# fgladwin/rocJPEG

Measured on NVIDIA B200. Metric: decoded_MP_per_s_rocJpegDecodeBatched, higher is better.
Workload: dtype u8 / int16 coefficients / int32 IDCT / fp32 colour

## Files before the change

### include/rocjpeg_b200_ext.h

```cpp
#ifndef ROCJPEG_B200_EXT_H
#define ROCJPEG_B200_EXT_H

#include <stddef.h>
#include <stdint.h>

#include "rocjpeg.h"

#if defined(__cplusplus)
extern "C" {
#endif

#define ROCJPEG_B200_STAGE_COUNT 7

typedef struct {
    float stage_ms[ROCJPEG_B200_STAGE_COUNT];
    float total_ms;
    uint32_t sync_rounds;
    uint32_t decodes_per_round[8];
    uint64_t scan_bytes;
    uint64_t blocks;
    uint64_t subsequences;
    uint64_t plane_bytes;
    uint64_t output_bytes;
    uint64_t h2d_bytes, d2h_bytes;
    uint32_t kernel_launches;
    int32_t subsequence_bytes;
    int32_t lanes;
    float host_submit_ms;
    float host_wait_ms;
    int32_t devices;
    uint64_t entries;
    uint32_t truncated_images;
    uint32_t pad_;
    uint64_t fused_blocks;
} RocJpegB200Stats;

RocJpegStatus rocJpegB200SetProfiling(RocJpegHandle handle, int enable);
RocJpegStatus rocJpegB200GetStats(RocJpegHandle handle, RocJpegB200Stats *stats);

RocJpegStatus rocJpegB200Prepare(RocJpegHandle handle, RocJpegStreamHandle *jpeg_stream_handles, int batch_size,
                                 const RocJpegDecodeParams *decode_params, RocJpegImage *destinations);
RocJpegStatus rocJpegB200Run(RocJpegHandle handle);

RocJpegStatus rocJpegB200GetScaledImageInfo(RocJpegHandle handle, RocJpegStreamHandle jpeg_stream_handle, int scale_denom, uint8_t *num_components,
                                            RocJpegChromaSubsampling *subsampling, uint32_t *widths, uint32_t *heights);
RocJpegStatus rocJpegB200DecodeBatchedScaled(RocJpegHandle handle, RocJpegStreamHandle *jpeg_stream_handles, int batch_size,
                                             const RocJpegDecodeParams *decode_params, const int32_t *scale_denoms, RocJpegImage *destinations);
RocJpegStatus rocJpegB200PrepareScaled(RocJpegHandle handle, RocJpegStreamHandle *jpeg_stream_handles, int batch_size,
                                       const RocJpegDecodeParams *decode_params, const int32_t *scale_denoms, RocJpegImage *destinations);

RocJpegStatus rocJpegB200ParseAndDecodeBatched(RocJpegHandle handle, RocJpegStreamHandle *jpeg_stream_handles,
                                               const unsigned char *const *datas, const size_t *lengths, int batch_size,
                                               const RocJpegDecodeParams *decode_params, RocJpegImage *destinations,
                                               double *parse_seconds);

RocJpegStatus rocJpegB200StreamLoadFiles(RocJpegStreamHandle *jpeg_stream_handles, const char *const *paths, int count,
                                         int io_threads, RocJpegStatus *per_file_status);

RocJpegStatus rocJpegB200GetCoefficients(RocJpegHandle handle, int index, int16_t *host_out, size_t count);
RocJpegStatus rocJpegB200GetPlanes(RocJpegHandle handle, int index, uint8_t *host_out, size_t count);

typedef struct {
    uint32_t segments_seen;
    uint32_t scan_size;
    uint32_t flags;
    uint32_t reserved;
} RocJpegB200ScanStatus;
#define ROCJPEG_B200_SCAN_NO_EOI 1u
#define ROCJPEG_B200_SCAN_STRAY_MARKER 2u
#define ROCJPEG_B200_SCAN_EXTRA_RESTARTS 4u
#define ROCJPEG_B200_SCAN_MISSING_INTERVALS 8u
#define ROCJPEG_B200_SCAN_EMPTY_INTERVAL 16u
#define ROCJPEG_B200_DECODE_SHORT 32u
#define ROCJPEG_B200_TRUNCATED_MASK (8u | 16u | 32u)
RocJpegStatus rocJpegB200GetScanStatus(RocJpegHandle handle, int index, RocJpegB200ScanStatus *status);
RocJpegStatus rocJpegB200GetImageStatus(RocJpegHandle handle, int index, uint32_t *flags);
RocJpegStatus rocJpegB200GetDeviceSegment(RocJpegHandle handle, int index, uint32_t segment, uint8_t *host_out, size_t capacity,
                                          uint32_t *nbytes);

typedef struct {
    int32_t width, height, num_components, chroma_subsampling;
    int32_t h_sampling[3], v_sampling[3], quant_selector[3], dc_selector[3], ac_selector[3];
    int32_t restart_interval;
    uint32_t num_mcus;
    uint32_t scan_offset;
    uint32_t raw_bytes;
    int32_t mcus_x, mcus_y, blocks_per_mcu;
    int32_t blocks_w[3], blocks_h[3];
    uint32_t num_segments;
    int32_t decode_status;
    int32_t source_is_device_visible;
    int32_t source_is_zero_copy;
    int32_t features;
} RocJpegB200StreamInfo;
#define ROCJPEG_B200_FEAT_SOF1 1
#define ROCJPEG_B200_FEAT_DQT16 2
#define ROCJPEG_B200_FEAT_HUFF_ID23 4
RocJpegStatus rocJpegB200StreamGetInfo(RocJpegStreamHandle jpeg_stream_handle, RocJpegB200StreamInfo *info);
typedef struct {
    uint32_t scan_size;
    uint32_t restart_markers_seen;
    uint32_t num_segments;
    uint64_t clean_bytes;
} RocJpegB200HostScanInfo;
RocJpegStatus rocJpegB200StreamHostScan(RocJpegStreamHandle jpeg_stream_handle, RocJpegB200HostScanInfo *info);
RocJpegStatus rocJpegB200StreamGetSegment(RocJpegStreamHandle jpeg_stream_handle, uint32_t segment, uint8_t *out,
                                          size_t capacity, uint32_t *nbytes);
RocJpegStatus rocJpegB200StreamGetLastError(RocJpegStreamHandle jpeg_stream_handle, char *out, size_t capacity);
RocJpegStatus rocJpegB200StreamGetQuantTable(RocJpegStreamHandle jpeg_stream_handle, int id, uint16_t out_natural[64]);
RocJpegStatus rocJpegB200StreamGetHuffmanTable(RocJpegStreamHandle jpeg_stream_handle, int is_ac, int id, uint8_t bits[16],
                                               uint8_t vals[256], uint32_t *count);

RocJpegStatus rocJpegB200PlanShards(const uint64_t *cost, int batch_size, int num_devices, int *out_device);
RocJpegStatus rocJpegB200PlanShardsPinned(const uint64_t *cost, const int *fixed, int batch_size, int num_devices, int *out_device);
RocJpegStatus rocJpegB200GetDeviceCount(RocJpegHandle handle, int *num_devices);

const char *rocJpegB200Version(void);
// ... 6 lines not shown
```

### rocjpeg_b200/api.py

```python
from __future__ import annotations

import ctypes as C
import os

HERE = os.path.dirname(os.path.abspath(__file__))
LIB_PATH = os.environ.get("ROCJPEG_B200_LIB") or os.path.join(HERE, "lib", "librocjpeg.so")

STATUS = {
    0: "ROCJPEG_STATUS_SUCCESS", -1: "ROCJPEG_STATUS_NOT_INITIALIZED", -2: "ROCJPEG_STATUS_INVALID_PARAMETER",
    -3: "ROCJPEG_STATUS_BAD_JPEG", -4: "ROCJPEG_STATUS_JPEG_NOT_SUPPORTED", -5: "ROCJPEG_STATUS_OUTOF_MEMORY",
    -6: "ROCJPEG_STATUS_EXECUTION_FAILED", -7: "ROCJPEG_STATUS_ARCH_MISMATCH", -8: "ROCJPEG_STATUS_INTERNAL_ERROR",
    -9: "ROCJPEG_STATUS_IMPLEMENTATION_NOT_SUPPORTED", -10: "ROCJPEG_STATUS_HW_JPEG_DECODER_NOT_SUPPORTED",
    -11: "ROCJPEG_STATUS_RUNTIME_ERROR", -12: "ROCJPEG_STATUS_NOT_IMPLEMENTED",
}
SUCCESS, NOT_INITIALIZED, INVALID_PARAMETER, BAD_JPEG, JPEG_NOT_SUPPORTED = 0, -1, -2, -3, -4
EXECUTION_FAILED, RUNTIME_ERROR, NOT_IMPLEMENTED = -6, -11, -12
CSS_444, CSS_440, CSS_422, CSS_420, CSS_411, CSS_400, CSS_UNKNOWN = 0, 1, 2, 3, 4, 5, -1
CSS_NAME = {0: "444", 1: "440", 2: "422", 3: "420", 4: "411", 5: "400", -1: "unknown"}
OUTPUT_NATIVE, OUTPUT_YUV_PLANAR, OUTPUT_Y, OUTPUT_RGB, OUTPUT_RGB_PLANAR = 0, 1, 2, 3, 4
FMT = {"native": 0, "yuv_planar": 1, "y": 2, "rgb": 3, "rgb_planar": 4}
BACKEND_HARDWARE, BACKEND_HYBRID = 0, 1
STAGES = ("upload", "destuff", "huffman_sync", "huffman_write", "dc", "idct", "output")


class RocJpegImage(C.Structure):
    _fields_ = [("channel", C.c_void_p * 4), ("pitch", C.c_uint32 * 4)]


class _Crop(C.Structure):
    _fields_ = [("left", C.c_int16), ("top", C.c_int16), ("right", C.c_int16), ("bottom", C.c_int16)]


class _Target(C.Structure):
    _fields_ = [("width", C.c_uint32), ("height", C.c_uint32)]


class RocJpegDecodeParams(C.Structure):
    _fields_ = [("output_format", C.c_int), ("crop_rectangle", _Crop), ("target_dimension", _Target)]


class Stats(C.Structure):
    _fields_ = [
        ("stage_ms", C.c_float * 7), ("total_ms", C.c_float), ("sync_rounds", C.c_uint32),
        ("decodes_per_round", C.c_uint32 * 8), ("scan_bytes", C.c_uint64), ("blocks", C.c_uint64),
        ("subsequences", C.c_uint64), ("plane_bytes", C.c_uint64), ("output_bytes", C.c_uint64),
        ("h2d_bytes", C.c_uint64), ("d2h_bytes", C.c_uint64), ("kernel_launches", C.c_uint32),
        ("subsequence_bytes", C.c_int32), ("lanes", C.c_int32),
        ("host_submit_ms", C.c_float), ("host_wait_ms", C.c_float), ("devices", C.c_int32),
        ("entries", C.c_uint64), ("truncated_images", C.c_uint32), ("pad_", C.c_uint32), ("fused_blocks", C.c_uint64),
    ]


class StreamInfo(C.Structure):
    _fields_ = [
        ("width", C.c_int32), ("height", C.c_int32), ("num_components", C.c_int32), ("chroma_subsampling", C.c_int32),
        ("h_sampling", C.c_int32 * 3), ("v_sampling", C.c_int32 * 3), ("quant_selector", C.c_int32 * 3),
        ("dc_selector", C.c_int32 * 3), ("ac_selector", C.c_int32 * 3), ("restart_interval", C.c_int32),
        ("num_mcus", C.c_uint32), ("scan_offset", C.c_uint32), ("raw_bytes", C.c_uint32),
        ("mcus_x", C.c_int32), ("mcus_y", C.c_int32), ("blocks_per_mcu", C.c_int32),
        ("blocks_w", C.c_int32 * 3), ("blocks_h", C.c_int32 * 3), ("num_segments", C.c_uint32),
        ("decode_status", C.c_int32), ("source_is_device_visible", C.c_int32), ("source_is_zero_copy", C.c_int32),
        ("features", C.c_int32),
    ]


class ScanStatus(C.Structure):
    _fields_ = [("segments_seen", C.c_uint32), ("scan_size", C.c_uint32), ("flags", C.c_uint32), ("reserved", C.c_uint32)]


FEAT_SOF1, FEAT_DQT16, FEAT_HUFF_ID23 = 1, 2, 4
SCAN_NO_EOI, SCAN_STRAY_MARKER, SCAN_EXTRA_RESTARTS, SCAN_MISSING_INTERVALS, SCAN_EMPTY_INTERVAL = 1, 2, 4, 8, 16
DECODE_SHORT, TRUNCATED_MASK = 32, 8 | 16 | 32


class HostScanInfo(C.Structure):
    _fields_ = [("scan_size", C.c_uint32), ("restart_markers_seen", C.c_uint32), ("num_segments", C.c_uint32),
                ("clean_bytes", C.c_uint64)]


EXPORTS = (
    "rocJpegStreamCreate", "rocJpegStreamParse", "rocJpegStreamDestroy", "rocJpegCreate", "rocJpegDestroy",
    "rocJpegGetImageInfo", "rocJpegDecode", "rocJpegDecodeBatched", "rocJpegGetErrorName",
)
EXT_EXPORTS = (
    "rocJpegB200SetProfiling", "rocJpegB200GetStats", "rocJpegB200Prepare", "rocJpegB200Run",
    "rocJpegB200GetCoefficients", "rocJpegB200GetPlanes", "rocJpegB200StreamGetInfo", "rocJpegB200StreamGetSegment",
    "rocJpegB200StreamGetQuantTable", "rocJpegB200StreamGetHuffmanTable", "rocJpegB200Version", "rocJpegB200StreamGetLastError",
    "rocJpegB200PlanShards", "rocJpegB200GetDeviceCount", "rocJpegB200StreamHostScan",
    "rocJpegB200GetScanStatus", "rocJpegB200GetDeviceSegment", "rocJpegB200ParseAndDecodeBatched",
    "rocJpegB200PlanShardsPinned", "rocJpegB200GetImageStatus", "rocJpegB200StreamLoadFiles",
    "rocJpegB200GetScaledImageInfo", "rocJpegB200DecodeBatchedScaled", "rocJpegB200PrepareScaled",
)
SCALES = (1, 2, 4, 8)

_lib = None


class RocJpegError(RuntimeError):
    def __init__(self, status: int, where: str):
        self.status = status
        super().__init__(f"{where}: {STATUS.get(status, status)}")


def load_library() -> C.CDLL:
    global _lib
    if _lib is not None:
        return _lib
    if not os.path.exists(LIB_PATH):
        raise RuntimeError(
            f"{LIB_PATH} is missing: build it with `make -C rocjpeg_b200/csrc` (or __graft_entry__.build()). "
            "rocjpeg_b200 has no CPU fallback.")
    L = C.CDLL(LIB_PATH)
    vp, i32 = C.c_void_p, C.c_int
    L.rocJpegStreamCreate.argtypes = [C.POINTER(vp)]
    L.rocJpegStreamParse.argtypes = [vp, C.c_size_t, vp]
    L.rocJpegStreamDestroy.argtypes = [vp]
    L.rocJpegCreate.argtypes = [i32, i32, C.POINTER(vp)]
    L.rocJpegDestroy.argtypes = [vp]
    L.rocJpegGetImageInfo.argtypes = [vp, vp, C.POINTER(C.c_uint8), C.POINTER(i32), C.POINTER(C.c_uint32), C.POINTER(C.c_uint32)]
    L.rocJpegDecode.argtypes = [vp, vp, C.POINTER(RocJpegDecodeParams), C.POINTER(RocJpegImage)]
    L.rocJpegDecodeBatched.argtypes = [vp, C.POINTER(vp), i32, C.POINTER(RocJpegDecodeParams), C.POINTER(RocJpegImage)]
    L.rocJpegGetErrorName.argtypes = [i32]
    L.rocJpegGetErrorName.restype = C.c_char_p
    L.rocJpegB200SetProfiling.argtypes = [vp, i32]
    L.rocJpegB200GetStats.argtypes = [vp, C.POINTER(Stats)]
    L.rocJpegB200Prepare.argtypes = [vp, C.POINTER(vp), i32, C.POINTER(RocJpegDecodeParams), C.POINTER(RocJpegImage)]
    L.rocJpegB200Run.argtypes = [vp]
    L.rocJpegB200GetScaledImageInfo.argtypes = [vp, vp, i32, C.POINTER(C.c_uint8), C.POINTER(i32), C.POINTER(C.c_uint32), C.POINTER(C.c_uint32)]
    L.rocJpegB200DecodeBatchedScaled.argtypes = [vp, C.POINTER(vp), i32, C.POINTER(RocJpegDecodeParams), C.POINTER(C.c_int32), C.POINTER(RocJpegImage)]
    L.rocJpegB200PrepareScaled.argtypes = [vp, C.POINTER(vp), i32, C.POINTER(RocJpegDecodeParams), C.POINTER(C.c_int32), C.POINTER(RocJpegImage)]
    L.rocJpegB200GetCoefficients.argtypes = [vp, i32, vp, C.c_size_t]
    L.rocJpegB200GetPlanes.argtypes = [vp, i32, vp, C.c_size_t]
# ... 287 lines not shown
```

### rocjpeg_b200/csrc/api.cpp

```cpp
#include <algorithm>
#include <atomic>
#include <chrono>
#include <thread>
#include <cstring>
#include <exception>
#include <iostream>
#include <memory>
#include <string>
#include <vector>

#include "decoder.h"
#include "jpeg_parser.h"
#include "rocjpeg_b200_ext.h"

#define ERR(X) std::cerr << "[ERR] " << " {" << __func__ << "} " << " " << X << std::endl;

namespace {

struct StreamHandle {
    std::shared_ptr<rjb::StreamParser> parser = std::make_shared<rjb::StreamParser>();
    std::string error;
};

struct DecoderHandle {
// ... 159 lines not shown
        ERR(e.what());
        return ROCJPEG_STATUS_RUNTIME_ERROR;
    }
}

RocJpegStatus ROCJPEGAPI rocJpegDecodeBatched(RocJpegHandle handle, RocJpegStreamHandle* jpeg_stream_handles, int batch_size,
                                              const RocJpegDecodeParams* decode_params, RocJpegImage* destinations) {
    return rocJpegB200DecodeBatchedScaled(handle, jpeg_stream_handles, batch_size, decode_params, nullptr, destinations);
}

RocJpegStatus rocJpegB200DecodeBatchedScaled(RocJpegHandle handle, RocJpegStreamHandle* jpeg_stream_handles, int batch_size,
                                             const RocJpegDecodeParams* decode_params, const int32_t* scale_denoms, RocJpegImage* destinations) {
    if (handle == nullptr || jpeg_stream_handles == nullptr || decode_params == nullptr || destinations == nullptr)
        return ROCJPEG_STATUS_INVALID_PARAMETER;
    auto h = static_cast<DecoderHandle*>(handle);
    try {
        if (batch_size < 0) return ROCJPEG_STATUS_INVALID_PARAMETER;
        std::vector<const rjb::StreamParser*> streams;
        int st = CollectStreams(jpeg_stream_handles, batch_size, &streams);
        if (st != 0) return RocJpegStatus(st);
        std::vector<rjb::DestImage> dsts;
        st = ToDests(destinations, batch_size, scale_denoms, &dsts);
        if (st != 0) return RocJpegStatus(st);
        st = h->decoder->Decode(streams.data(), batch_size, ToParams(decode_params), dsts.data());
        if (st != 0) h->CaptureError(h->decoder->last_error());
        return RocJpegStatus(st);
    } catch (const std::exception& e) {
        h->CaptureError(e.what());
        ERR(e.what());
        return ROCJPEG_STATUS_RUNTIME_ERROR;
    }
}

const char* ROCJPEGAPI rocJpegGetErrorName(RocJpegStatus rocjpeg_status) {
    switch (rocjpeg_status) {
        case ROCJPEG_STATUS_SUCCESS: return "ROCJPEG_STATUS_SUCCESS";
        case ROCJPEG_STATUS_NOT_INITIALIZED: return "ROCJPEG_STATUS_NOT_INITIALIZED";
        case ROCJPEG_STATUS_INVALID_PARAMETER: return "ROCJPEG_STATUS_INVALID_PARAMETER";
        case ROCJPEG_STATUS_BAD_JPEG: return "ROCJPEG_STATUS_BAD_JPEG";
        case ROCJPEG_STATUS_JPEG_NOT_SUPPORTED: return "ROCJPEG_STATUS_JPEG_NOT_SUPPORTED";
        case ROCJPEG_STATUS_EXECUTION_FAILED: return "ROCJPEG_STATUS_EXECUTION_FAILED";
        case ROCJPEG_STATUS_ARCH_MISMATCH: return "ROCJPEG_STATUS_ARCH_MISMATCH";
        case ROCJPEG_STATUS_INTERNAL_ERROR: return "ROCJPEG_STATUS_INTERNAL_ERROR";
        case ROCJPEG_STATUS_IMPLEMENTATION_NOT_SUPPORTED: return "ROCJPEG_STATUS_IMPLEMENTATION_NOT_SUPPORTED";
        case ROCJPEG_STATUS_HW_JPEG_DECODER_NOT_SUPPORTED: return "ROCJPEG_STATUS_HW_JPEG_DECODER_NOT_SUPPORTED";
        case ROCJPEG_STATUS_RUNTIME_ERROR: return "ROCJPEG_STATUS_RUNTIME_ERROR";
        case ROCJPEG_STATUS_OUTOF_MEMORY: return "ROCJPEG_STATUS_OUTOF_MEMORY";
        case ROCJPEG_STATUS_NOT_IMPLEMENTED: return "ROCJPEG_STATUS_NOT_IMPLEMENTED";
        default: return "UNKNOWN_ERROR";
    }
}


RocJpegStatus rocJpegB200SetProfiling(RocJpegHandle handle, int enable) {
    if (handle == nullptr) return ROCJPEG_STATUS_INVALID_PARAMETER;
    static_cast<DecoderHandle*>(handle)->decoder->SetProfiling(enable);
    return ROCJPEG_STATUS_SUCCESS;
}

RocJpegStatus rocJpegB200GetStats(RocJpegHandle handle, RocJpegB200Stats* stats) {
    if (handle == nullptr || stats == nullptr) return ROCJPEG_STATUS_INVALID_PARAMETER;
    const rjb::BatchStats& s = static_cast<DecoderHandle*>(handle)->decoder->stats();
    std::memset(stats, 0, sizeof(*stats));
    for (int i = 0; i < ROCJPEG_B200_STAGE_COUNT; i++) stats->stage_ms[i] = s.stage_ms[i];
    stats->total_ms = s.total_ms;
    stats->sync_rounds = s.sync_rounds;
    for (int i = 0; i < 8; i++) stats->decodes_per_round[i] = s.decodes_per_round[i];
    stats->scan_bytes = s.scan_bytes;
    stats->blocks = s.blocks;
    stats->subsequences = s.subsequences;
    stats->plane_bytes = s.plane_bytes;
    stats->output_bytes = s.output_bytes;
    stats->h2d_bytes = s.h2d_bytes;
    stats->d2h_bytes = s.d2h_bytes;
    stats->kernel_launches = s.kernel_launches;
    stats->subsequence_bytes = s.sub_bytes;
    stats->lanes = s.lanes;
    stats->host_submit_ms = s.host_submit_ms;
    stats->host_wait_ms = s.host_wait_ms;
    stats->devices = s.devices;
    stats->entries = s.entries;
    stats->truncated_images = s.truncated_images;
    stats->fused_blocks = s.fused_blocks;
    return ROCJPEG_STATUS_SUCCESS;
}

RocJpegStatus rocJpegB200Prepare(RocJpegHandle handle, RocJpegStreamHandle* jpeg_stream_handles, int batch_size,
                                 const RocJpegDecodeParams* decode_params, RocJpegImage* destinations) {
    return rocJpegB200PrepareScaled(handle, jpeg_stream_handles, batch_size, decode_params, nullptr, destinations);
}

RocJpegStatus rocJpegB200PrepareScaled(RocJpegHandle handle, RocJpegStreamHandle* jpeg_stream_handles, int batch_size,
                                       const RocJpegDecodeParams* decode_params, const int32_t* scale_denoms, RocJpegImage* destinations) {
    if (handle == nullptr || jpeg_stream_handles == nullptr || decode_params == nullptr || destinations == nullptr || batch_size <= 0)
        return ROCJPEG_STATUS_INVALID_PARAMETER;
    auto h = static_cast<DecoderHandle*>(handle);
    try {
        std::vector<const rjb::StreamParser*> streams;
        int st = CollectStreams(jpeg_stream_handles, batch_size, &streams);
        if (st != 0) return RocJpegStatus(st);
        std::vector<rjb::DestImage> dsts;
        st = ToDests(destinations, batch_size, scale_denoms, &dsts);
        if (st != 0) return RocJpegStatus(st);
        return RocJpegStatus(h->decoder->Prepare(streams.data(), batch_size, ToParams(decode_params), dsts.data()));
    } catch (const std::exception& e) {
        h->CaptureError(e.what());
        ERR(e.what());
        return ROCJPEG_STATUS_RUNTIME_ERROR;
    }
}

RocJpegStatus rocJpegB200Run(RocJpegHandle handle) {
    if (handle == nullptr) return ROCJPEG_STATUS_INVALID_PARAMETER;
    auto h = static_cast<DecoderHandle*>(handle);
    try {
        return RocJpegStatus(h->decoder->Run());
    } catch (const std::exception& e) {
        h->CaptureError(e.what());
        ERR(e.what());
        return ROCJPEG_STATUS_RUNTIME_ERROR;
    }
}

RocJpegStatus rocJpegB200ParseAndDecodeBatched(RocJpegHandle handle, RocJpegStreamHandle* jpeg_stream_handles, const unsigned char* const* datas,
                                               const size_t* lengths, int batch_size, const RocJpegDecodeParams* decode_params,
                                               RocJpegImage* destinations, double* parse_seconds) {
    if (handle == nullptr || jpeg_stream_handles == nullptr || datas == nullptr || lengths == nullptr || batch_size < 0)
        return ROCJPEG_STATUS_INVALID_PARAMETER;
    const auto t0 = std::chrono::steady_clock::now();
    for (int i = 0; i < batch_size; i++) {
        const RocJpegStatus st = rocJpegStreamParse(datas[i], lengths[i], jpeg_stream_handles[i]);
        if (st != ROCJPEG_STATUS_SUCCESS) return st;
    }
    if (parse_seconds) *parse_seconds = std::chrono::duration<double>(std::chrono::steady_clock::now() - t0).count();
    return rocJpegDecodeBatched(handle, jpeg_stream_handles, batch_size, decode_params, destinations);
}

RocJpegStatus rocJpegB200StreamLoadFiles(RocJpegStreamHandle* jpeg_stream_handles, const char* const* paths, int count, int io_threads,
                                         RocJpegStatus* per_file_status) {
    if (jpeg_stream_handles == nullptr || paths == nullptr || count < 0) return ROCJPEG_STATUS_INVALID_PARAMETER;
    for (int i = 0; i < count; i++)
        if (jpeg_stream_handles[i] == nullptr || paths[i] == nullptr) return ROCJPEG_STATUS_INVALID_PARAMETER;
    const int nthreads = std::max(1, std::min(io_threads <= 0 ? 8 : io_threads, std::max(count, 1)));
    std::vector<RocJpegStatus> status(size_t(count), ROCJPEG_STATUS_SUCCESS);
    std::atomic<int> next{0};
    auto work = [&]() {
        for (;;) {
            const int i = next.fetch_add(1, std::memory_order_relaxed);
            if (i >= count) return;
            auto h = static_cast<StreamHandle*>(jpeg_stream_handles[i]);
            try {
                const int rc = h->parser->ParseFile(paths[i]);
                h->error = rc == 0 ? std::string() : h->parser->last_error();
                status[size_t(i)] = rc == 0 ? ROCJPEG_STATUS_SUCCESS : rc == -2 ? ROCJPEG_STATUS_INVALID_PARAMETER : ROCJPEG_STATUS_BAD_JPEG;
            } catch (const std::exception& e) {
                h->error = e.what();
                status[size_t(i)] = ROCJPEG_STATUS_RUNTIME_ERROR;
            }
        }
    };
    std::vector<std::thread> pool;
    for (int t = 1; t < nthreads; t++) pool.emplace_back(work);
    work();
    for (auto& t : pool) t.join();
    RocJpegStatus first = ROCJPEG_STATUS_SUCCESS;
    for (int i = 0; i < count; i++) {
// ... 150 lines not shown
```

### rocjpeg_b200/csrc/decoder.cpp

```cpp
#include "decoder.h"

#include "huff_core.cuh"

#include <cuda_runtime.h>

#include <algorithm>
#include <chrono>
#include <cstdint>
#include <cstdio>
#include <cstdlib>
#include <cstring>
#include <iostream>

namespace rjb {

namespace {
constexpr int kSuccess = 0, kNotInitialized = -1, kInvalidParameter = -2, kBadJpeg = -3, kNotSupported = -4,
              kOutOfMemory = -5, kExecutionFailed = -6, kNotImplemented = -12;

inline size_t AlignUp(size_t v, size_t a) { return (v + a - 1) / a * a; }

int EnvInt(const char* name, int dflt) {
    const char* v = std::getenv(name);
    return (v && *v) ? std::atoi(v) : dflt;
// ... 498 lines not shown
        raw_off += AlignUp(size_t(up_bytes) + 16, 128);
        im.k0_tile0 = k0tile;
        h_k0_tile0_[size_t(i)] = k0tile;
        k0tile += std::max<uint32_t>(1u, uint32_t((size_t(im.raw_skip) + rs.nbytes + kK0TileBytes - 1) / kK0TileBytes));
        im.data_off = scan_off;
        im.seg0 = nseg_total;
        im.nseg = p.nseg;
        {
            const uint64_t mcus = uint64_t(im.total_mcus);
            h_needed_segments_[size_t(i)] = p.restart_interval > 0 ? uint32_t((mcus + uint32_t(p.restart_interval) - 1) / uint32_t(p.restart_interval)) : 1u;
        }
        nseg_total += p.nseg;
        const uint64_t clean_cap = CleanCapacity(rs.nbytes, p.nseg, uint32_t(S));
        scan_off += clean_cap;
        im.sub0 = uint32_t(sub);
        im.nsub = uint32_t(clean_cap / uint32_t(S));
        sub = AlignUp(sub + im.nsub, owned);
        if (sub > 0x7FFFFFFFull || nseg_total > 0x7FFFFFFFu) return Fail(kNotSupported, "batch too large for one decode call");
        h_img_cta0_[size_t(i)] = im.sub0 / owned;
        im.seg_keep_lo = 0;
        im.seg_keep_hi = 0xFFFFFFFFu;
        {
            const uint32_t cw = uint32_t(int(params.crop_right) - int(params.crop_left));
            const uint32_t chh = uint32_t(int(params.crop_bottom) - int(params.crop_top));
            if (p.restart_interval > 0 && cw > 0 && chh > 0 && cw <= uint32_t(out_w) && chh <= uint32_t(out_h) &&
                params.crop_top >= 0 && params.crop_bottom <= out_h && im.mcus_y > 0) {
                const int mcu_h = 8 * std::max(1, p.ncomp == 1 ? 1 : p.vmax) / d;
                const uint64_t row_lo = uint64_t(params.crop_top / mcu_h), row_hi = uint64_t((params.crop_bottom - 1) / mcu_h);
                const uint64_t ri = uint64_t(p.restart_interval);
                const uint64_t k_lo = row_lo * uint64_t(im.mcus_x) / ri, k_hi = ((row_hi + 1) * uint64_t(im.mcus_x) - 1) / ri;
                im.seg_keep_lo = uint32_t(k_lo > 0 ? k_lo - 1 : 0);
                im.seg_keep_hi = uint32_t(std::min<uint64_t>(k_hi, 0xFFFFFFFFull));
            }
        }
        im.blk0 = blk;
        im.nblocks = uint32_t(im.total_mcus) * uint32_t(p.bpm);
        blk += im.nblocks;
        im.ent0 = ent;
        const uint64_t ent_cap = uint64_t(rs.nbytes) * 8 / p.min_entry_bits + 7 * (uint64_t(im.nsub) + 1) + 64;
        if (ent_cap > 0xFFFFFF00ull) return Fail(kNotSupported, "scan too large for one picture");
        im.ent_cap = uint32_t(ent_cap);
        ent += (uint64_t(im.ent_cap) + 63) & ~uint64_t(63);
        im.dc_tile0 = dctile;
        h_img_dctile0_[size_t(i)] = dctile;
        dctile += uint32_t((im.total_mcus + kDcTileMcus - 1) / kDcTileMcus);
        h_k2_tile0_[size_t(i)] = k2tile;
        for (int s = 0; s < kScaledKernels; s++) h_k2s_tile0_[s][size_t(i)] = k2stile[s];
        uint32_t& idct_tiles = d == 1 ? k2tile : k2stile[ScaleIndex(d)];
        const int bs = 8 / d;
        for (int c = 0; c < p.ncomp; c++) {
            im.plane_pitch[c] = uint32_t(AlignUp(size_t(p.blocks_w[c]) * bs, 64));
            im.plane_off[c] = plane_off;
            plane_off += AlignUp(size_t(im.plane_pitch[c]) * size_t(p.blocks_h[c]) * bs, 256);
            idct_tiles += uint32_t((p.blocks_w[c] + 31) / 32) * uint32_t(p.blocks_h[c]);
            stats_.plane_bytes += uint64_t(p.blocks_w[c]) * p.blocks_h[c] * uint64_t(bs * bs);
        }
        OutputDesc& od = h_outputs_[size_t(i)];
        const uint32_t rw = uint32_t(int(params.crop_right) - int(params.crop_left));
        const uint32_t rh = uint32_t(int(params.crop_bottom) - int(params.crop_top));
        od.x0 = od.y0 = 0;
        od.w = out_w;
        od.h = out_h;
        if (rw > 0 && rh > 0 && rw <= uint32_t(out_w) && rh <= uint32_t(out_h)) {
            if (params.crop_left < 0 || params.crop_top < 0 || params.crop_right > out_w || params.crop_bottom > out_h)
                return Fail(kInvalidParameter, "crop rectangle lies outside the picture");
            od.x0 = params.crop_left; od.y0 = params.crop_top; od.w = int32_t(rw); od.h = int32_t(rh);
        }
        od.fmt = params.output_format;
        for (int c = 0; c < 4; c++) {
            od.dst[c] = dsts[i].channel[c];
            od.dst_pitch[c] = dsts[i].pitch[c];
        }
        const bool whole = od.x0 == 0 && od.y0 == 0 && od.w == out_w && od.h == out_h;
        const bool planar = od.fmt == FMT_Y || od.fmt == FMT_YUV_PLANAR ||
                            (od.fmt == FMT_NATIVE && (p.css == CSS_444 || p.css == CSS_440 || p.css == CSS_411 || p.css == CSS_400));
        od.direct = (whole && planar && direct_ok && !(remote && remote[i])) ? 1 : 0;
        od.fused = (d == 1 && whole && fuse_ok && (od.fmt == FMT_RGB || od.fmt == FMT_RGB_PLANAR) && h_fused_.size() < 65535) ? 1 : 0;
        const bool tiles = !od.direct && !od.fused;
        od.tiles_x = tiles ? uint32_t((od.w + kK3TileW - 1) / kK3TileW) : 0u;
        od.tiles_y = tiles ? uint32_t((od.h + kK3TileH - 1) / kK3TileH) : 0u;
        any_direct_ = any_direct_ || od.direct || od.fused || !whole;
        needs_planes_ = needs_planes_ || tiles;
        k2_needed_ = k2_needed_ || (!od.fused && d == 1);
        if (od.fused) {
            FusedImage fi = {};
            fi.ent0 = im.ent0; fi.blk0 = im.blk0; fi.ent_cap = im.ent_cap;
            for (int c = 0; c < 3; c++) fi.dst[c] = od.dst[c];
            fi.dpitch = od.dst_pitch[0];
            fi.width = p.width; fi.height = p.height; fi.css = p.css; fi.fmt = od.fmt;
            fi.ncomp = p.ncomp; fi.bpm = p.bpm; fi.mcus_x = p.mcus_x;
            int hmax = 1, vmax = 1;
            for (int c = 0; c < p.ncomp; c++) { hmax = std::max(hmax, im.hs[c]); vmax = std::max(vmax, im.vs[c]); }
            fi.vmax = vmax;
            fi.mpt = kK3TileW / (8 * hmax);
            fi.tiles_x = uint32_t((p.width + kK3TileW - 1) / kK3TileW);
            bool aligned = (od.dst_pitch[0] & 3u) == 0;
            for (int c = 0; c < (od.fmt == FMT_RGB ? 1 : 3); c++) aligned = aligned && (reinterpret_cast<uintptr_t>(od.dst[c]) & 3u) == 0;
            aligned = aligned && warp_ok && (fi.mpt / 8) * p.bpm <= 16;
            if (remote && remote[i]) aligned = false;
            fi.tile0 = aligned ? k23tile_w : k23tile;
            fi.sx = p.css == CSS_411 ? 2 : (p.css == CSS_422 || p.css == CSS_420) ? 1 : 0;
            fi.sy = (p.css == CSS_440 || p.css == CSS_420) ? 1 : 0;
            uint32_t off = 0;
            for (int c = 0; c < p.ncomp; c++) {
                fi.H[c] = uint8_t(im.hs[c]); fi.V[c] = uint8_t(im.vs[c]); fi.first_blk[c] = uint8_t(im.comp_first_blk[c]);
                fi.hshift[c] = uint8_t(im.hs[c] == 4 ? 2 : im.hs[c] == 2 ? 1 : 0);
                fi.qidx[c] = uint32_t(im.qt_index[c]);
                fi.pitch[c] = uint32_t(8 * fi.mpt * im.hs[c]);
                fi.base[c] = off;
                fi.comp_info[c] = uint32_t(fi.H[c]) | (uint32_t(fi.V[c]) << 8) | (uint32_t(fi.first_blk[c]) << 16) | (uint32_t(fi.hshift[c]) << 24);
                off += c == 0 ? 16u * kK3TileW : 8u * kK3TileW;
            }
            const uint32_t ntiles = fi.tiles_x * uint32_t(p.mcus_y);
            std::vector<uint32_t>& list = aligned ? h_tile_img_w_ : h_tile_img_;
            for (uint32_t r = 0; r < uint32_t(p.mcus_y); r++) list.insert(list.end(), fi.tiles_x, uint32_t(h_fused_.size()) | (r << 16));
            h_fused_.push_back(fi);
            (aligned ? k23tile_w : k23tile) += ntiles;
            stats_.fused_blocks += im.nblocks;
        }
        od.tile0 = k3tile;
        h_k3_tile0_[size_t(i)] = k3tile;
        k3tile += od.tiles_x * od.tiles_y;
        stats_.output_bytes += OutputBytes(p.css, od.fmt, od.w, od.h);
    }
    h_img_cta0_[size_t(n)] = uint32_t(sub / owned);
    h_k0_tile0_[size_t(n)] = k0tile;
    h_img_dctile0_[size_t(n)] = dctile;
    h_k2_tile0_[size_t(n)] = k2tile;
    for (int s = 0; s < kScaledKernels; s++) h_k2s_tile0_[s][size_t(n)] = k2stile[s];
    h_k3_tile0_[size_t(n)] = k3tile;
    scan_bytes_ = scan_off;
    raw_bytes_ = raw_off;
    if (!h_runs_.empty()) raw_bytes_ = AlignUp(size_t(h_runs_.back().dst_off) + h_runs_.back().nbytes + 16, 128);
    nseg_total_ = nseg_total;
    coef_blocks_ = blk;
    entry_count_ = ent;
    plane_bytes_ = plane_off;
    nsub_total_ = sub;
    stats_.scan_bytes = total_clean;
    stats_.blocks = blk;
    stats_.subsequences = sub;

    k1_ = K1Args{};
    k1_.nimages = n;
    k1_.total_ctas = uint32_t(sub / owned);
    k1_.halo = halo;
    k0_ = K0Args{};
    k0_.nimages = n;
    k0_.total_tiles = k0tile;
    k0_.sub_bytes = S;
    {
        uint32_t most_tiles = 0;
        for (int i = 0; i < n; i++) most_tiles = std::max(most_tiles, h_k0_tile0_[size_t(i) + 1] - h_k0_tile0_[size_t(i)]);
        k0_.inline_scan = (most_tiles <= 32u && EnvInt("ROCJPEG_B200_NO_INLINE_SCAN", 0) == 0) ? 1 : 0;
    }
    k1_.rec_fill_vecs = uint32_t((blk * sizeof(BlockRec) + 15) / 16);
    k1_.lut_smem_bytes = max_pairs * 2u * uint32_t(kFastSize) * 4u + max_sub * 4u;
    k1_.total_dc_tiles = dctile;
    k1_.sub_bytes = S;
    {
        uint32_t most = 0;
        for (int i = 0; i < n; i++) most = std::max(most, h_img_cta0_[size_t(i) + 1] - h_img_cta0_[size_t(i)]);
        k1_.inline_scan = (most <= 32u && EnvInt("ROCJPEG_B200_NO_INLINE_SCAN", 0) == 0) ? 1 : 0;
        k1_.fusable = most <= uint32_t(std::max(0, EnvInt("ROCJPEG_B200_K1_FUSE_CTAS", 256))) ? 1 : 0;
        uint32_t most_mcus = 0;
        for (int i = 0; i < n; i++) most_mcus = std::max(most_mcus, uint32_t(h_images_[size_t(i)].total_mcus));
        const int dc_limit = EnvInt("ROCJPEG_B200_DC_IMAGE_MCUS", n >= 16 ? 2 * kDcImageMaxMcus : kDcImageMaxMcus);
        k1_.dc_image = (most_mcus <= uint32_t(std::max(0, dc_limit)) && EnvInt("ROCJPEG_B200_NO_DC_IMAGE", 0) == 0) ? 1 : 0;
    }
    k2_ = K2Args{};
    k2_.nimages = n;
    k2_.total_tiles = k2tile;
    for (int s = 0; s < kScaledKernels; s++) {
        k2s_[s] = K2Args{};
        k2s_[s].nimages = n;
        k2s_[s].total_tiles = k2stile[s];
    }
    k3_ = K3Args{};
    k3_.nimages = n;
    k3_.total_tiles = k3tile;
    k23_ = K23Args{};
    k23_.nimages = n;
    k23_.total_tiles = k23tile;
    k23_.total_tiles_w = k23tile_w;
    return kSuccess;
}

struct Lane::Layout {
    size_t images, outputs, cta0, k0tile0, dctile0, k2tile0, k2stile0[kScaledKernels], k3tile0, fused, tile_img, tile_img_w, gather, luts, qtables, total;
};

int Lane::Upload(cudaStream_t up, UploadTurn turn) {
    TurnGuard guard(turn);
    if (up == nullptr) up = stream_;
    const size_t n = h_images_.size();
    Layout L;
    size_t o = 0;
    auto place = [&](size_t bytes) { size_t at = o; o = AlignUp(o + bytes, 256); return at; };
    L.images = place(n * sizeof(ImageDesc));
    L.outputs = place(n * sizeof(OutputDesc));
    L.cta0 = place((n + 1) * 4);
    L.k0tile0 = place((n + 1) * 4);
    L.dctile0 = place((n + 1) * 4);
    L.k2tile0 = place((n + 1) * 4);
    for (int s = 0; s < kScaledKernels; s++) L.k2stile0[s] = place((n + 1) * 4);
    L.k3tile0 = place((n + 1) * 4);
    L.fused = place(h_fused_.size() * sizeof(FusedImage));
    L.tile_img = place(h_tile_img_.size() * 4);
    L.tile_img_w = place(h_tile_img_w_.size() * 4);
    L.gather = place(n * sizeof(GatherItem));
    L.luts = place(h_lut_ptrs_.size() * sizeof(HuffLutSet));
    L.qtables = place(h_qtables_.size() * 2);
    L.total = o;
    uint8_t* h = h_desc_.Reserve(L.total);
    if (!h) return Fail(kOutOfMemory, "descriptor staging");
    std::memcpy(h + L.images, h_images_.data(), n * sizeof(ImageDesc));
    std::memcpy(h + L.outputs, h_outputs_.data(), n * sizeof(OutputDesc));
    std::memcpy(h + L.cta0, h_img_cta0_.data(), (n + 1) * 4);
    std::memcpy(h + L.k0tile0, h_k0_tile0_.data(), (n + 1) * 4);
    std::memcpy(h + L.dctile0, h_img_dctile0_.data(), (n + 1) * 4);
    std::memcpy(h + L.k2tile0, h_k2_tile0_.data(), (n + 1) * 4);
    for (int s = 0; s < kScaledKernels; s++) std::memcpy(h + L.k2stile0[s], h_k2s_tile0_[s].data(), (n + 1) * 4);
    std::memcpy(h + L.k3tile0, h_k3_tile0_.data(), (n + 1) * 4);
    std::memcpy(h + L.fused, h_fused_.data(), h_fused_.size() * sizeof(FusedImage));
    std::memcpy(h + L.tile_img, h_tile_img_.data(), h_tile_img_.size() * 4);
    std::memcpy(h + L.tile_img_w, h_tile_img_w_.data(), h_tile_img_w_.size() * 4);
    std::memcpy(h + L.gather, h_gather_.data(), n * sizeof(GatherItem));
    for (size_t s = 0; s < h_lut_ptrs_.size(); s++) std::memcpy(h + L.luts + s * sizeof(HuffLutSet), h_lut_ptrs_[s], sizeof(HuffLutSet));
    std::memcpy(h + L.qtables, h_qtables_.data(), h_qtables_.size() * 2);
    desc_bytes_ = L.total;

    size_t off = 0;
    auto carve = [&](size_t bytes) { const size_t at = off; off = AlignUp(off + bytes + 256, 256); return at; };
    const size_t o_desc = carve(L.total), o_raw = carve(raw_bytes_ + 512), o_scan = carve(scan_bytes_ + 512),
                 o_segments = carve(size_t(nseg_total_) * sizeof(SegmentDesc)), o_tile_sum = carve(size_t(k0_.total_tiles) * 16),
                 o_tile_carry = carve(size_t(k0_.total_tiles) * 16), o_status = carve(n * sizeof(ScanStatus)), o_entries = carve(entry_count_ * 4),
                 o_blkrec = carve(coef_blocks_ * sizeof(BlockRec)), o_nnz = carve(nsub_total_ * 4), o_state = carve(nsub_total_ * 4),
                 o_used = carve(nsub_total_ * 4), o_subseg = carve(nsub_total_ * 4), o_cta_entries = carve(size_t(k1_.total_ctas) * 4),
                 o_cta_partial = carve(size_t(k1_.total_ctas) * 8), o_cta_carry = carve(size_t(k1_.total_ctas) * 8), o_cta_flag = carve(size_t(k1_.total_ctas) * 8 + 4),
                 o_cta_dc = carve(size_t(k1_.total_ctas) * 32),
                 o_dc_partial = carve(size_t(k1_.total_dc_tiles) * 12), o_dc_carry = carve(size_t(k1_.total_dc_tiles) * 12),
                 o_end = carve(0);
    (void)o_end;
    RJB_CUDA(d_slab_.Reserve(off));
    if (needs_planes_) RJB_CUDA(d_planes_.Reserve(plane_bytes_ + 512));
    if (!h_counters_.Reserve(256 + n * sizeof(ScanStatus))) return Fail(kOutOfMemory, "counter staging");

    uint8_t* base = d_slab_.as<uint8_t>();
    uint8_t* d = base + o_desc;
    k1_.images = reinterpret_cast<const ImageDesc*>(d + L.images);
    k1_.segments = reinterpret_cast<const SegmentDesc*>(base + o_segments);
    k0_.images = k1_.images;
    k0_.segments = reinterpret_cast<SegmentDesc*>(base + o_segments);
    k0_.img_tile0 = reinterpret_cast<const uint32_t*>(d + L.k0tile0);
    k0_.raw = base + o_raw;
    k0_.clean = base + o_scan;
    k0_.tile_sum = reinterpret_cast<uint4*>(base + o_tile_sum);
    k0_.tile_carry = reinterpret_cast<uint4*>(base + o_tile_carry);
    k0_.status = reinterpret_cast<ScanStatus*>(base + o_status);
    k1_.status = k0_.status;
    k1_.img_cta0 = reinterpret_cast<const uint32_t*>(d + L.cta0);
    k1_.img_dctile0 = reinterpret_cast<const uint32_t*>(d + L.dctile0);
    k1_.scan = base + o_scan;
    k1_.luts = reinterpret_cast<const HuffLutSet*>(d + L.luts);
    k1_.state = reinterpret_cast<uint32_t*>(base + o_state);
    k1_.used = reinterpret_cast<uint32_t*>(base + o_used);
    k1_.sub_seg = reinterpret_cast<uint32_t*>(base + o_subseg);
    k1_.cta_partial = reinterpret_cast<uint2*>(base + o_cta_partial);
    k1_.dc_partial = reinterpret_cast<int3*>(base + o_dc_partial);
    k1_.dc_carry = reinterpret_cast<int3*>(base + o_dc_carry);
    k1_.cta_carry = reinterpret_cast<uint2*>(base + o_cta_carry);
    k1_.cta_flag = reinterpret_cast<uint32_t*>(base + o_cta_flag);
    k1_.cta_dc = reinterpret_cast<int4*>(base + o_cta_dc);
    k1_.entries = reinterpret_cast<uint32_t*>(base + o_entries);
    k1_.blk_rec = reinterpret_cast<BlockRec*>(base + o_blkrec);
    k1_.nnz = reinterpret_cast<uint32_t*>(base + o_nnz);
    k1_.cta_entries = reinterpret_cast<uint32_t*>(base + o_cta_entries);
    k2_.images = k1_.images;
    k2_.outputs = reinterpret_cast<const OutputDesc*>(d + L.outputs);
    k2_.force_planes = 0;
    k2_.img_tile0 = reinterpret_cast<const uint32_t*>(d + L.k2tile0);
    k2_.qtables = reinterpret_cast<const uint16_t*>(d + L.qtables);
    k2_.entries = k1_.entries;
    k2_.blk_rec = k1_.blk_rec;
    k2_.planes = needs_planes_ ? d_planes_.as<uint8_t>() : nullptr;
    for (int s = 0; s < kScaledKernels; s++) {
        const uint32_t tiles = k2s_[s].total_tiles;
        k2s_[s] = k2_;
        k2s_[s].img_tile0 = reinterpret_cast<const uint32_t*>(d + L.k2stile0[s]);
        k2s_[s].total_tiles = tiles;
    }
    k3_.images = k1_.images;
    k3_.outputs = reinterpret_cast<const OutputDesc*>(d + L.outputs);
    k3_.img_tile0 = reinterpret_cast<const uint32_t*>(d + L.k3tile0);
    k3_.planes = k2_.planes;
    k23_.fused = reinterpret_cast<const FusedImage*>(d + L.fused);
    k23_.tile_img = reinterpret_cast<const uint32_t*>(d + L.tile_img);
    k23_.tile_img_w = reinterpret_cast<const uint32_t*>(d + L.tile_img_w);
    k23_.qtables = k2_.qtables;
    k23_.entries = k1_.entries;
    k23_.blk_rec = k1_.blk_rec;

    guard.Acquire();
    host_ms_[1] = NowMs();
    if (ev_trace_[0]) RJB_CUDA(cudaEventRecord(ev_trace_[0], up));
    RJB_CUDA(cudaMemcpyAsync(d, h, L.total, cudaMemcpyHostToDevice, up));
    stats_.h2d_bytes = L.total;
    for (const GatherItem& g : h_gather_) stats_.h2d_bytes += g.nbytes;
    const bool use_runs = !h_runs_.empty();
    const bool use_gather = !use_runs && all_pinned_ && h_images_.size() > 4 && raw_bytes_ / h_images_.size() < (256u << 10) &&
                            EnvInt("ROCJPEG_B200_NO_GATHER", 0) == 0;
    tiles_reduced_ = use_gather;
    if (use_gather) {
        RJB_CUDA(LaunchGatherReduce(k0_, reinterpret_cast<const GatherItem*>(d + L.gather), up));
        stats_.kernel_launches++;
    } else if (use_runs) {
        stats_.h2d_bytes = L.total;
        for (const CopyRun& r : h_runs_) {
            RJB_CUDA(cudaMemcpyAsync(const_cast<uint8_t*>(k0_.raw) + r.dst_off, r.src, r.nbytes, cudaMemcpyHostToDevice, up));
            stats_.h2d_bytes += r.nbytes;
        }
    } else {
        for (size_t i = 0; i < n; i++)
            RJB_CUDA(cudaMemcpyAsync(const_cast<uint8_t*>(k0_.raw) + h_gather_[i].dst_off, h_gather_[i].src, h_gather_[i].nbytes,
                                     cudaMemcpyHostToDevice, up));
    }
    if (ev_trace_[1]) RJB_CUDA(cudaEventRecord(ev_trace_[1], up));
    if (up != stream_) {
        RJB_CUDA(cudaEventRecord(ev_uploaded_, up));
        guard.Release();
        RJB_CUDA(cudaStreamWaitEvent(stream_, ev_uploaded_, 0));
    }
    return kSuccess;
}

int Lane::LaunchAll(bool include_upload, int profiling_, cudaStream_t up, UploadTurn turn) {
    const int rounds = std::min(std::max(EnvInt("ROCJPEG_B200_SYNC_ROUNDS", 2), 1), kMaxSyncRounds);
    static const bool debug_sync = EnvInt("ROCJPEG_B200_DEBUG_SYNC", 0) != 0;
    auto mark = [&](int i) -> cudaError_t {
        if (debug_sync) {
            const cudaError_t e = cudaStreamSynchronize(stream_);
            if (e != cudaSuccess) {
                static const char* const kNames[] = {"(before)", "upload", "destuff", "huffman sync", "huffman write", "dc", "idct", "output"};
                std::cerr << "[rocjpeg_b200] stage '" << kNames[i] << "' failed: " << cudaGetErrorName(e) << std::endl;
                return e;
            }
        }
        const bool want = profiling_ == 1 || (profiling_ == 2 && (i == 0 || i == kStageCount));
        return want ? cudaEventRecord(ev_[i], stream_) : cudaSuccess;
    };
    stats_.kernel_launches = 0;
    struct ExitGuard {
        Lane* lane;
        TurnGuard turn;
        bool ok = false;
        ~ExitGuard() {
            if (!ok && lane->d_counters_.capacity() >= 512) cudaMemsetAsync(lane->d_counters_.as<uint8_t>(), 0, 512, lane->stream_);
        }
    } exit_guard{this, TurnGuard(include_upload ? turn : UploadTurn())};
    RJB_CUDA(mark(0));
    if (include_upload) {
        exit_guard.turn.passed = true;
        int st = Upload(up, turn);
        if (st != kSuccess) return st;
    }
    RJB_CUDA(mark(1));
    k1_.counters = d_counters_.as<uint32_t>() + 64 * counter_set_;
    k1_.counters_next = d_counters_.as<uint32_t>() + 64 * (counter_set_ ^ 1);
    counter_set_ ^= 1;
    if (k1_.total_ctas == 0) {
        RJB_CUDA(cudaMemsetAsync(k1_.blk_rec, 0xFF, coef_blocks_ * sizeof(BlockRec), stream_));
        RJB_CUDA(cudaMemsetAsync(k1_.counters_next, 0, 256, stream_));
    }
    const bool k1_fuse_ok = EnvInt("ROCJPEG_B200_NO_K1_FUSE", 0) == 0 && std::getenv("ROCJPEG_B200_SYNC_ROUNDS") == nullptr;
    const bool k1_fused = k1_fuse_ok && k1_.fusable && k1_.total_ctas != 0;
    k1_.k1_dc = k1_fused && k1_.dc_image && EnvInt("ROCJPEG_B200_NO_K1_DC", 0) == 0 ? 1 : 0;
    if (k1_fused) RJB_CUDA(cudaMemsetAsync(k1_.cta_flag, 0, size_t(k1_.total_ctas) * 8 + 4, stream_));
    if (!(include_upload && tiles_reduced_)) {
        RJB_CUDA(LaunchK0Reduce(k0_, stream_));
        stats_.kernel_launches++;
    }
    RJB_CUDA(LaunchK0Destuff(k0_, stream_));
    stats_.kernel_launches += k0_.inline_scan ? 1 : 2;
    RJB_CUDA(mark(2));
    if (k1_fused) {
        RJB_CUDA(LaunchK1Fused(k1_, stream_));
        stats_.sync_rounds = 1;
        RJB_CUDA(mark(3));
    } else {
        for (int r = 0; r < rounds; r++) RJB_CUDA(LaunchK1Sync(k1_, r, stream_));
        stats_.sync_rounds = uint32_t(rounds);
        RJB_CUDA(mark(3));
        RJB_CUDA(LaunchK1Write(k1_, stream_));
    }
    RJB_CUDA(mark(4));
    if (!k1_.k1_dc) RJB_CUDA(LaunchDcScan(k1_, stream_));
    RJB_CUDA(mark(5));
    uint32_t idct_launches = 0;
    {
        const int st = LaunchIdct(false, &idct_launches);
        if (st != kSuccess) return st;
    }
    RJB_CUDA(mark(6));
    RJB_CUDA(LaunchK23Fused(k23_, stream_));
    RJB_CUDA(LaunchK3Output(k3_, stream_));
    RJB_CUDA(mark(7));
    stats_.kernel_launches += (k1_fused ? 1u : uint32_t(rounds) + (k1_.inline_scan ? 1u : 2u)) + (k1_.k1_dc ? 0 : k1_.dc_image ? 1 : 3) + idct_launches +
                              (k23_.total_tiles ? 1 : 0) + (k23_.total_tiles_w ? 1 : 0) +
                              (k3_.total_tiles ? 1 : 0);
    RJB_CUDA(cudaMemcpyAsync(h_counters_.data(), k1_.counters, 256, cudaMemcpyDeviceToHost, stream_));
    RJB_CUDA(cudaMemcpyAsync(h_counters_.data() + 256, k0_.status, h_images_.size() * sizeof(ScanStatus), cudaMemcpyDeviceToHost, stream_));
    stats_.d2h_bytes = 256 + h_images_.size() * sizeof(ScanStatus);
    if (ev_trace_[2]) RJB_CUDA(cudaEventRecord(ev_trace_[2], stream_));
    host_ms_[2] = NowMs();
    exit_guard.ok = true;
    return kSuccess;
}

int Lane::LaunchIdct(bool force_planes, uint32_t* launches) {
    K2Args k2 = k2_;
    k2.force_planes = force_planes ? 1 : 0;
    if (k2_needed_ || force_planes) {
        RJB_CUDA(LaunchK2Idct(k2, stream_));
        if (k2.total_tiles) (*launches)++;
    }
    for (int s = 0; s < kScaledKernels; s++) {
        K2Args ks = k2s_[s];
        ks.force_planes = k2.force_planes;
        RJB_CUDA(LaunchK2Scaled(ks, 2 << s, stream_));
        if (ks.total_tiles) (*launches)++;
    }
    return kSuccess;
}

int Lane::Finish(int profiling_) {
    RJB_CUDA(cudaStreamSynchronize(stream_));
    const uint32_t* cnt = reinterpret_cast<const uint32_t*>(h_counters_.data());
    uint32_t last = stats_.sync_rounds - 1;
    if (cnt[last] != 0) {
        uint32_t guard = 0;
        for (;;) {
            uint32_t slot = std::min<uint32_t>(last + 1, kMaxSyncRounds - 1);
            RJB_CUDA(cudaMemsetAsync(k1_.counters + slot, 0, 4, stream_));
            RJB_CUDA(LaunchK1Sync(k1_, int(slot), stream_));
            RJB_CUDA(cudaMemcpyAsync(h_counters_.data(), k1_.counters, 256, cudaMemcpyDeviceToHost, stream_));
            RJB_CUDA(cudaStreamSynchronize(stream_));
            stats_.sync_rounds++;
            stats_.kernel_launches++;
            last = slot;
            if (cnt[slot] == 0) break;
            if (++guard > k1_.total_ctas + 2) return Fail(kExecutionFailed, "entropy decoder failed to converge");
        }
        RJB_CUDA(cudaMemsetAsync(k1_.blk_rec, 0xFF, coef_blocks_ * sizeof(BlockRec), stream_));
        RJB_CUDA(cudaMemsetAsync(k1_.counters + 2 * kMaxSyncRounds, 0, 4, stream_));
        RJB_CUDA(LaunchK1ClearShort(k1_, stream_));
        RJB_CUDA(LaunchK1Write(k1_, stream_));
        RJB_CUDA(LaunchDcScan(k1_, stream_));
        uint32_t idct_launches = 0;
        const int st = LaunchIdct(false, &idct_launches);
        if (st != kSuccess) return st;
        RJB_CUDA(LaunchK23Fused(k23_, stream_));
        RJB_CUDA(LaunchK3Output(k3_, stream_));
        RJB_CUDA(cudaMemcpyAsync(h_counters_.data(), k1_.counters, 256, cudaMemcpyDeviceToHost, stream_));
        RJB_CUDA(cudaMemcpyAsync(h_counters_.data() + 256, k0_.status, h_images_.size() * sizeof(ScanStatus), cudaMemcpyDeviceToHost, stream_));
        RJB_CUDA(cudaStreamSynchronize(stream_));
        stats_.kernel_launches += 8;
    }
    stats_.entries = cnt[2 * kMaxSyncRounds];
    ScanStatus* st = reinterpret_cast<ScanStatus*>(h_counters_.data() + 256);
    truncated_images_ = 0;
    for (size_t i = 0; i < h_images_.size(); i++) {
        if (st[i].segments_seen < h_needed_segments_[i]) st[i].flags |= kScanMissingIntervals;
        if (st[i].flags & kStatusTruncatedMask) truncated_images_++;
    }
    for (int r = 0; r < kMaxSyncRounds; r++) stats_.decodes_per_round[r] = cnt[kMaxSyncRounds + r];
    if (profiling_) {
        for (int s = 0; s < kStageCount && profiling_ == 1; s++) {
            float ms = 0;
            if (cudaEventElapsedTime(&ms, ev_[s], ev_[s + 1]) == cudaSuccess) stats_.stage_ms[s] = ms;
        }
        float ms = 0;
        if (cudaEventElapsedTime(&ms, ev_[0], ev_[kStageCount]) == cudaSuccess) stats_.total_ms = ms;
        (void)cudaGetLastError();
    }
    return kSuccess;
}

void Lane::PrintTimeline(int index, cudaEvent_t origin, double host_origin_ms) const {
    float t[3] = {-1, -1, -1};
    for (int i = 0; i < 3; i++)
        if (ev_trace_[i] && origin && cudaEventElapsedTime(&t[i], origin, ev_trace_[i]) != cudaSuccess) (void)cudaGetLastError();
    std::fprintf(stderr, "[rocjpeg_b200]   lane %d: %zu images, %zu raw bytes | host: describe %.3f, enqueue %.3f .. %.3f ms | device: upload %.3f .. %.3f, done %.3f ms\n",
                 index, h_images_.size(), raw_bytes_, host_ms_[0] - host_origin_ms, host_ms_[1] - host_origin_ms, host_ms_[2] - host_origin_ms, t[0], t[1], t[2]);
}

int Decoder::Split(const StreamParser* const* streams, int n) {
    uint64_t total = 0;
    for (int i = 0; i < n; i++) total += streams[i] ? streams[i]->parsed().raw_bytes : 0;
    int want = EnvInt("ROCJPEG_B200_LANES", 0);
    if (want <= 0) {
        want = int(std::min<uint64_t>(4, total / (2u << 20)));
        if (n > 0 && total / uint64_t(n) >= (256u << 10)) want = std::max(want, int(std::min<uint64_t>(kMaxLanes, total / (8u << 20))));
    }
    want = std::max(1, std::min(std::min(want, kMaxLanes), n));
    double cum[kMaxLanes + 1] = {0};
    for (int l = 1; l <= want; l++) cum[l] = double(l) / want;
    if (want == 4 && n > 0 && total / uint64_t(n) < (256u << 10)) {
        cum[1] = 0.20; cum[2] = 0.50; cum[3] = 0.80; cum[4] = 1.0;
    }
    if (const char* sp = std::getenv("ROCJPEG_B200_SPLIT")) {
        double w[kMaxLanes] = {0}, sum = 0;
        int k = 0;
        for (const char* q = sp; *q && k < want;) {
            w[k] = std::max(0.0, std::atof(q));
            sum += w[k++];
            while (*q && *q != ',') q++;
            if (*q == ',') q++;
        }
        if (k == want && sum > 0) {
            double run = 0;
            for (int l = 0; l < want; l++) cum[l + 1] = (run += w[l]) / sum;
        }
    }
    uint64_t acc = 0;
    int lane = 0;
    chunk_first_[0] = 0;
    for (int i = 0; i < n && lane + 1 < want; i++) {
        acc += streams[i] ? streams[i]->parsed().raw_bytes : 0;
        if (double(acc) >= double(total) * cum[lane + 1] && i + 1 < n) chunk_first_[++lane] = i + 1;
    }
    active_lanes_ = lane + 1;
    chunk_first_[active_lanes_] = n;
    return active_lanes_;
}

int Decoder::BuildAll(const StreamParser* const* streams, int n, const DecodeParams& params, const DestImage* dsts, bool launch, const uint8_t* remote) {
    for (int i = 0; i < n; i++) {
        if (!streams[i]) return Fail(kInvalidParameter, "null stream handle in batch");
        const ParsedJpeg& p = streams[i]->parsed();
        if (!p.valid) return Fail(kBadJpeg, "stream handle holds no successfully parsed JPEG");
        if (p.support_status != kSuccess) {
            if (p.support_status == kNotSupported)
                std::cerr << "[ERR]  {Decode}  The JPEG image (chroma subsampling / layout / size) is not supported!" << std::endl;
            return Fail(p.support_status, "unsupported or inconsistent JPEG");
        }
        const int d = dsts[i].scale_denom;
        if (!ValidScale(d)) return Fail(kInvalidParameter, "scale denominator must be 1, 2, 4 or 8");
        const int out_w = (p.width + d - 1) / d, out_h = (p.height + d - 1) / d;
        const uint32_t rw = uint32_t(int(params.crop_right) - int(params.crop_left));
        const uint32_t rh = uint32_t(int(params.crop_bottom) - int(params.crop_top));
        if (rw > 0 && rh > 0 && rw <= uint32_t(out_w) && rh <= uint32_t(out_h) &&
// ... 6 lines not shown
    for (int l = 0; l < active_lanes_; l++) {
        const int st = lanes_[l].Create(device_id_, sm_count_, l < 4);
        if (st != kSuccess) return Fail(st, lanes_[l].last_error());
    }
    const bool threaded = active_lanes_ > 1 && EnvInt("ROCJPEG_B200_SUBMIT_THREADS", 0) != 0;
    std::atomic<int> turn{0};
    int status[kMaxLanes] = {};
    bool any_pending = false;
    for (int i = 0; i < n && !any_pending; i++) any_pending = streams[i]->staging_pending();
    auto stage = [&](int l) {
        const int first = chunk_first_[l], cnt = chunk_first_[l + 1] - first;
        const int threads = std::min(std::max(1, EnvInt("ROCJPEG_B200_COPY_THREADS", 4)), std::min(cnt, kMaxLanes));
        if (threads <= 1) {
            for (int i = first; i < first + cnt; i++) streams[i]->EnsureStaged();
            return;
        }
        if (!pool_) pool_.reset(new SubmitPool(kMaxLanes - 1));
        pool_->Run(threads, [&](int t) {
            for (int i = first + t; i < first + cnt; i += threads) streams[i]->EnsureStaged();
        });
    };
    auto submit = [&](int l) {
        DeviceGuard guard(device_id_);
        Lane& lane = lanes_[l];
        const int first = chunk_first_[l], cnt = chunk_first_[l + 1] - first;
        UploadTurn ut;
        ut.turn = threaded ? &turn : nullptr;
        ut.mine = l;
        lane.set_host_mark(0, NowMs());
        int st = lane.Build(streams + first, cnt, params, dsts + first, remote ? remote + first : nullptr);
        if (st == kSuccess) st = launch ? lane.LaunchAll(true, profiling_, upload_stream_, ut) : lane.Upload(upload_stream_, ut);
        else TurnGuard pass(ut);
        status[l] = st;
    };
    if (threaded) {
        for (int l = 0; l < active_lanes_ && any_pending; l++) stage(l);
        if (!pool_) pool_.reset(new SubmitPool(kMaxLanes - 1));
        pool_->Run(active_lanes_, submit);
    } else {
        for (int l = 0; l < active_lanes_; l++) {
            if (any_pending) stage(l);
            submit(l);
            if (status[l] != kSuccess) break;
        }
    }
    for (int l = 0; l < active_lanes_; l++) {
        if (status[l] != kSuccess) {
            for (int k = 0; k < active_lanes_; k++) lanes_[k].Sync();
            return Fail(status[l], lanes_[l].last_error());
        }
    }
    return kSuccess;
}

int Decoder::FinishAll() {
    int status = kSuccess;
    uint32_t truncated = 0;
    for (int l = 0; l < active_lanes_; l++) {
        int st = lanes_[l].Finish(profiling_);
        if (st != kSuccess && status == kSuccess) status = Fail(st, lanes_[l].last_error());
        truncated += lanes_[l].truncated_images();
    }
    Aggregate();
    stats_.truncated_images = truncated;
    if (status == kSuccess && truncated != 0 && strict_status_)
        status = Fail(kBadJpeg, std::to_string(truncated) + " picture(s) of the batch ended before their last block (truncated or damaged scan)");
    return status;
}

void Decoder::Aggregate() {
    stats_ = BatchStats();
    stats_.lanes = active_lanes_;
    for (int l = 0; l < active_lanes_; l++) {
        const BatchStats& s = lanes_[l].stats();
        for (int i = 0; i < kStageCount; i++) stats_.stage_ms[i] += s.stage_ms[i];
        stats_.sync_rounds = std::max(stats_.sync_rounds, s.sync_rounds);
        for (int r = 0; r < kMaxSyncRounds; r++) stats_.decodes_per_round[r] += s.decodes_per_round[r];
        stats_.scan_bytes += s.scan_bytes;
        stats_.blocks += s.blocks;
        stats_.entries += s.entries;
        stats_.subsequences += s.subsequences;
        stats_.plane_bytes += s.plane_bytes;
        stats_.fused_blocks += s.fused_blocks;
        stats_.output_bytes += s.output_bytes;
        stats_.h2d_bytes += s.h2d_bytes;
        stats_.d2h_bytes += s.d2h_bytes;
        stats_.kernel_launches += s.kernel_launches;
        stats_.sub_bytes = std::max(stats_.sub_bytes, s.sub_bytes);
        if (profiling_) {
            float ms = 0;
            if (cudaEventElapsedTime(&ms, lanes_[0].first_event(), lanes_[l].last_event()) == cudaSuccess)
                stats_.total_ms = std::max(stats_.total_ms, ms);
            (void)cudaGetLastError();
        }
    }
}

int Decoder::Decode(const StreamParser* const* streams, int n, const DecodeParams& params, const DestImage* dsts) {
    std::lock_guard<std::mutex> lock(mutex_);
    if (!initialized_) return Fail(kNotInitialized, "decoder not initialised");
    if (!streams || !dsts || n < 0) return kInvalidParameter;
    if (n == 0) return kSuccess;
    sharded_ = false;
    if (!peers_.empty() && n >= 2) return DecodeSharded(streams, n, params, dsts);
    DeviceGuard guard(device_id_);
    prepared_ = false;
    const auto t0 = std::chrono::steady_clock::now();
    int st = BuildAll(streams, n, params, dsts, true);
    if (st != kSuccess) return st;
    const auto t1 = std::chrono::steady_clock::now();
    st = FinishAll();
    const auto t2 = std::chrono::steady_clock::now();
    stats_.host_submit_ms = std::chrono::duration<float, std::milli>(t1 - t0).count();
    stats_.host_wait_ms = std::chrono::duration<float, std::milli>(t2 - t1).count();
    if (TraceLevel()) {
        std::cerr << "[rocjpeg_b200] decode n=" << n << " lanes=" << active_lanes_ << " submit_ms=" << stats_.host_submit_ms
                  << " wait_ms=" << stats_.host_wait_ms << std::endl;
        const double origin = std::chrono::duration<double, std::milli>(t0.time_since_epoch()).count();
        for (int l = 0; l < active_lanes_ && TraceLevel() >= 2; l++) lanes_[l].PrintTimeline(l, lanes_[0].trace_origin(), origin);
    }
    prepared_ = (st == kSuccess) || (st == kBadJpeg && stats_.truncated_images != 0);
    return st;
}

int Decoder::Submit(const StreamParser* const* streams, int n, const DecodeParams& params, const DestImage* dsts, const uint8_t* remote) {
    DeviceGuard guard(device_id_);
    prepared_ = false;
    return BuildAll(streams, n, params, dsts, true, remote);
}

int Decoder::Wait() {
    DeviceGuard guard(device_id_);
    int st = FinishAll();
    prepared_ = (st == kSuccess) || (st == kBadJpeg && stats_.truncated_images != 0);
    return st;
}

int Decoder::DecodeSharded(const StreamParser* const* streams, int n, const DecodeParams& params, const DestImage* dsts) {
    const auto t0 = std::chrono::steady_clock::now();
    const int ndev = 1 + int(peers_.size());
    std::vector<uint64_t> cost(static_cast<size_t>(n), 0);
    for (int i = 0; i < n; i++) {
        if (!streams[i]) return Fail(kInvalidParameter, "null stream handle in batch");
        const ParsedJpeg& p = streams[i]->parsed();
        if (!p.valid) return Fail(kBadJpeg, "stream handle holds no successfully parsed JPEG");
        if (p.support_status != kSuccess) return Fail(p.support_status, "unsupported or inconsistent JPEG");
        cost[size_t(i)] = p.raw_bytes;
    }
    std::vector<int> fixed(static_cast<size_t>(n), -1), owner(static_cast<size_t>(n), 0);
    uintptr_t range_base = 0;
    size_t range_size = 0;
    int range_dev = -1;
    for (int i = 0; i < n; i++) {
        const uintptr_t ptr = reinterpret_cast<uintptr_t>(dsts[i].channel[0]);
        if (!(range_size != 0 && ptr >= range_base && ptr - range_base < range_size))
            range_dev = DeviceOfPointer(dsts[i].channel[0], &range_base, &range_size);
        const int dev = range_dev;
        for (int d = 1; d < ndev; d++)
            if (dev == peers_[size_t(d - 1)]->device_id()) fixed[size_t(i)] = d;
        if (dev >= 0 && dev != device_id_ && fixed[size_t(i)] < 0)
            return Fail(kInvalidParameter, "destination buffer on a device this handle does not drive");
        owner[size_t(i)] = fixed[size_t(i)] >= 0 ? fixed[size_t(i)] : 0;
    }
    shard_dev_.assign(size_t(n), 0);
    shard_local_.assign(size_t(n), 0);
    PlanShardsPinned(cost.data(), fixed.data(), n, ndev, shard_dev_.data());
    std::vector<std::vector<const StreamParser*>> sub_streams(static_cast<size_t>(ndev));
    std::vector<std::vector<DestImage>> sub_dsts(static_cast<size_t>(ndev));
    std::vector<std::vector<uint8_t>> sub_remote(static_cast<size_t>(ndev));
    for (int i = 0; i < n; i++) {
        const size_t d = size_t(shard_dev_[size_t(i)]);
        shard_local_[size_t(i)] = int(sub_streams[d].size());
        sub_streams[d].push_back(streams[i]);
        sub_dsts[d].push_back(dsts[i]);
        sub_remote[d].push_back(uint8_t(int(d) != owner[size_t(i)] ? 1 : 0));
    }
    int status = kSuccess;
    std::vector<char> submitted(static_cast<size_t>(ndev), 0);
    std::vector<int> sub_status(static_cast<size_t>(ndev), kSuccess);
    auto submit = [&](int d) {
        if (sub_streams[size_t(d)].empty()) return;
        Decoder* dec = d == 0 ? this : peers_[size_t(d - 1)].get();
        sub_status[size_t(d)] = dec->Submit(sub_streams[size_t(d)].data(), int(sub_streams[size_t(d)].size()), params, sub_dsts[size_t(d)].data(),
                                             sub_remote[size_t(d)].data());
        submitted[size_t(d)] = sub_status[size_t(d)] == kSuccess ? 1 : 0;
    };
    if (!shard_pool_) shard_pool_.reset(new SubmitPool(ndev - 1));
    shard_pool_->Run(ndev, submit);
    for (int d = 0; d < ndev; d++)
        if (sub_status[size_t(d)] != kSuccess && status == kSuccess)
            status = Fail(sub_status[size_t(d)], (d == 0 ? this : peers_[size_t(d - 1)].get())->last_error());
    const auto t1 = std::chrono::steady_clock::now();
    BatchStats total;
    total.devices = 0;
    for (int d = 0; d < ndev; d++) {
        if (!submitted[size_t(d)]) continue;
        Decoder* dec = d == 0 ? this : peers_[size_t(d - 1)].get();
        const int st = dec->Wait();
        if (st != kSuccess && status == kSuccess) status = Fail(st, dec->last_error());
        const BatchStats& s = dec->stats_;
        for (int i = 0; i < kStageCount; i++) total.stage_ms[i] += s.stage_ms[i];
        total.total_ms = std::max(total.total_ms, s.total_ms);
        total.sync_rounds = std::max(total.sync_rounds, s.sync_rounds);
        for (int r = 0; r < kMaxSyncRounds; r++) total.decodes_per_round[r] += s.decodes_per_round[r];
        total.scan_bytes += s.scan_bytes;
        total.blocks += s.blocks;
        total.entries += s.entries;
        total.truncated_images += s.truncated_images;
        total.subsequences += s.subsequences;
        total.plane_bytes += s.plane_bytes;
        total.fused_blocks += s.fused_blocks;
        total.output_bytes += s.output_bytes;
        total.h2d_bytes += s.h2d_bytes;
        total.d2h_bytes += s.d2h_bytes;
        total.kernel_launches += s.kernel_launches;
        total.sub_bytes = std::max(total.sub_bytes, s.sub_bytes);
        total.lanes += s.lanes;
        total.devices++;
    }
    const auto t2 = std::chrono::steady_clock::now();
    stats_ = total;
    stats_.host_submit_ms = std::chrono::duration<float, std::milli>(t1 - t0).count();
    stats_.host_wait_ms = std::chrono::duration<float, std::milli>(t2 - t1).count();
    sharded_ = (status == kSuccess) || (status == kBadJpeg && total.truncated_images != 0);
    if (status != kSuccess) prepared_ = false;
    return status;
}

int Decoder::Prepare(const StreamParser* const* streams, int n, const DecodeParams& params, const DestImage* dsts) {
    std::lock_guard<std::mutex> lock(mutex_);
    if (!initialized_) return Fail(kNotInitialized, "decoder not initialised");
    if (!streams || !dsts || n <= 0) return kInvalidParameter;
    DeviceGuard guard(device_id_);
    prepared_ = false;
    int st = BuildAll(streams, n, params, dsts, false);
    if (st != kSuccess) return st;
    for (int l = 0; l < active_lanes_; l++) {
        st = lanes_[l].Sync();
        if (st != kSuccess) return Fail(st, lanes_[l].last_error());
    }
    prepared_ = true;
    return kSuccess;
}

int Decoder::Run() {
    std::lock_guard<std::mutex> lock(mutex_);
    if (!initialized_ || !prepared_) return Fail(kNotInitialized, "no prepared batch");
    DeviceGuard guard(device_id_);
    for (int l = 0; l < active_lanes_; l++) {
        int st = lanes_[l].LaunchAll(false, profiling_, nullptr);
        if (st != kSuccess) return Fail(st, lanes_[l].last_error());
    }
    return FinishAll();
}

Lane* Decoder::Locate(int image, int* local) {
    if (sharded_) {
        if (image < 0 || size_t(image) >= shard_dev_.size()) return nullptr;
        const int d = shard_dev_[size_t(image)];
        if (d > 0) return peers_[size_t(d - 1)]->Locate(shard_local_[size_t(image)], local);
        image = shard_local_[size_t(image)];
    }
    if (!prepared_ || image < 0 || image >= chunk_first_[active_lanes_]) return nullptr;
    int l = 0;
    while (image >= chunk_first_[l + 1]) l++;
    *local = image - chunk_first_[l];
    return &lanes_[l];
}

int Decoder::CopyCoefficients(int image, int16_t* host_out, size_t count) {
    std::lock_guard<std::mutex> lock(mutex_);
    int local = 0;
    Lane* lane = host_out ? Locate(image, &local) : nullptr;
    if (!lane) return kInvalidParameter;
    return lane->CopyCoefficients(local, host_out, count);
}

int Decoder::CopyPlanes(int image, uint8_t* host_out, size_t count) {
    std::lock_guard<std::mutex> lock(mutex_);
    int local = 0;
    Lane* lane = host_out ? Locate(image, &local) : nullptr;
    if (!lane) return kInvalidParameter;
    return lane->CopyPlanes(local, host_out, count);
}

int Decoder::CopySegment(int image, uint32_t segment, uint8_t* host_out, size_t capacity, uint32_t* nbytes) {
    std::lock_guard<std::mutex> lock(mutex_);
    int local = 0;
    Lane* lane = nbytes ? Locate(image, &local) : nullptr;
    if (!lane) return kInvalidParameter;
    return lane->CopySegment(local, segment, host_out, capacity, nbytes);
}

int Decoder::GetScanStatus(int image, ScanStatus* out) {
// ... 93 lines not shown
```

### rocjpeg_b200/csrc/decoder.h

```cpp
#pragma once
#include <cuda_runtime_api.h>

#include <atomic>
#include <condition_variable>
#include <cstdint>
#include <functional>
#include <memory>
#include <mutex>
#include <string>
#include <thread>
#include <vector>

#include "device_types.h"
#include "jpeg_parser.h"
#include "stages.h"

namespace rjb {

struct DecodeParams {
    int32_t output_format;
    int16_t crop_left, crop_top, crop_right, crop_bottom;
};
struct DestImage {
    uint8_t* channel[4];
    uint32_t pitch[4];
    int32_t scale_denom;
};
constexpr int kScaledKernels = 3;
inline bool ValidScale(int d) { return d == 1 || d == 2 || d == 4 || d == 8; }
inline int ScaleIndex(int d) { return d == 2 ? 0 : d == 4 ? 1 : 2; }

class DeviceBuffer {
  public:
    DeviceBuffer() = default;
    ~DeviceBuffer();
    DeviceBuffer(const DeviceBuffer&) = delete;
    DeviceBuffer& operator=(const DeviceBuffer&) = delete;
    cudaError_t Reserve(size_t bytes);
    template <class U> U* as() const { return reinterpret_cast<U*>(ptr_); }
    size_t capacity() const { return cap_; }

  private:
    void* ptr_ = nullptr;
    size_t cap_ = 0;
};

enum StageId {
    kStageUpload = 0,
    kStageDestuff,
    kStageSync,
    kStageWrite,
    kStageDc,
    kStageIdct,
    kStageOutput,
    kStageCount
};

struct BatchStats {
    float stage_ms[kStageCount] = {};
    float total_ms = 0;
    uint32_t sync_rounds = 0;
    uint32_t decodes_per_round[kMaxSyncRounds] = {};
    uint64_t scan_bytes = 0;
    uint64_t blocks = 0;
    uint64_t entries = 0;
    uint64_t subsequences = 0;
    uint64_t plane_bytes = 0;
    uint64_t fused_blocks = 0;
    uint64_t output_bytes = 0;
    uint64_t h2d_bytes = 0, d2h_bytes = 0;
    uint32_t kernel_launches = 0;
    int sub_bytes = 0;
    int lanes = 0;
    float host_submit_ms = 0, host_wait_ms = 0;
    int devices = 1;
    uint32_t truncated_images = 0;
};

class SubmitPool {
  public:
    explicit SubmitPool(int workers);
    ~SubmitPool();
    SubmitPool(const SubmitPool&) = delete;
    SubmitPool& operator=(const SubmitPool&) = delete;
    void Run(int n, const std::function<void(int)>& fn);

  private:
    void Loop(int index);
    std::vector<std::thread> threads_;
    std::mutex m_;
    std::condition_variable cv_;
    uint64_t generation_ = 0;
    int jobs_ = 0;
    const std::function<void(int)>* fn_ = nullptr;
    std::atomic<int> pending_{0};
    bool stop_ = false;
};

struct UploadTurn {
    std::atomic<int>* turn = nullptr;
    int mine = 0;
};

class Lane {
  public:
    Lane() = default;
    ~Lane();
    Lane(const Lane&) = delete;
    Lane& operator=(const Lane&) = delete;
    int Create(int device_id, int sm_count, bool prealloc = true);
    int Build(const StreamParser* const* streams, int n, const DecodeParams& params, const DestImage* dsts, const uint8_t* remote = nullptr);
    int Upload(cudaStream_t upload_stream, UploadTurn turn = UploadTurn());
    int LaunchAll(bool include_upload, int profiling, cudaStream_t upload_stream, UploadTurn turn = UploadTurn());
    int Finish(int profiling);
    int Sync();
    int CopyCoefficients(int image, int16_t* host_out, size_t count);
    int CopyPlanes(int image, uint8_t* host_out, size_t count);
    int CopySegment(int image, uint32_t segment, uint8_t* host_out, size_t capacity, uint32_t* nbytes);
    int GetScanStatus(int image, ScanStatus* out) const;
    const BatchStats& stats() const { return stats_; }
    const std::string& last_error() const { return err_; }
    cudaEvent_t first_event() const { return ev_[0]; }
    cudaEvent_t last_event() const { return ev_[kStageCount]; }
    int num_images() const { return int(h_images_.size()); }
    uint32_t truncated_images() const { return truncated_images_; }
    void PrintTimeline(int index, cudaEvent_t origin, double host_origin_ms) const;
    cudaEvent_t trace_origin() const { return ev_trace_[0]; }
    void set_host_mark(int i, double ms) { host_ms_[i] = ms; }

  private:
    struct Layout;
    int Fail(int status, const std::string& why);
    int LaunchIdct(bool force_planes, uint32_t* launches);

    bool created_ = false;
    std::string err_;
    cudaStream_t stream_ = nullptr;
    cudaEvent_t ev_[kStageCount + 1] = {};
    cudaEvent_t ev_uploaded_ = nullptr;
    cudaEvent_t ev_trace_[3] = {};
    double host_ms_[3] = {};
    int sm_count_ = 0;

    std::vector<ImageDesc> h_images_;
    std::vector<OutputDesc> h_outputs_;
    std::vector<uint32_t> h_img_cta0_, h_img_dctile0_, h_k2_tile0_, h_k3_tile0_, h_k0_tile0_, h_needed_segments_;
    std::vector<uint32_t> h_k2s_tile0_[kScaledKernels];
    std::vector<int> h_scale_;
    uint32_t truncated_images_ = 0;
    std::vector<GatherItem> h_gather_;
    struct CopyRun {
        const uint8_t* src;
        uint64_t dst_off;
        size_t nbytes;
    };
    std::vector<CopyRun> h_runs_;
    std::vector<FusedImage> h_fused_;
    std::vector<uint32_t> h_tile_img_;
    std::vector<uint32_t> h_tile_img_w_;
    std::vector<const HuffLutSet*> h_lut_ptrs_;
    std::vector<const ParsedJpeg*> h_lut_specs_;
    std::vector<uint64_t> h_lut_hashes_;
    std::vector<uint16_t> h_qtables_;
    K0Args k0_ = {};
    K1Args k1_ = {};
    K2Args k2_ = {};
    K2Args k2s_[kScaledKernels] = {};
    K3Args k3_ = {};
    K23Args k23_ = {};
    bool k2_needed_ = true;
    bool tiles_reduced_ = false;
    bool all_pinned_ = false, any_direct_ = false, needs_planes_ = false;
    size_t scan_bytes_ = 0, raw_bytes_ = 0, coef_blocks_ = 0, entry_count_ = 0, plane_bytes_ = 0, nsub_total_ = 0;
    uint32_t nseg_total_ = 0;

    StagingBuffer h_desc_;
    size_t desc_bytes_ = 0;
    StagingBuffer h_counters_;
    DeviceBuffer d_slab_;
    DeviceBuffer d_planes_;
    DeviceBuffer d_counters_;
    int counter_set_ = 0;
    BatchStats stats_;
};

constexpr int kMaxLanes = 8;
constexpr int kMaxDevices = 16;



void PlanShards(const uint64_t* cost, int n, int ndev, int* out_device);
void PlanShardsPinned(const uint64_t* cost, const int* fixed, int n, int ndev, int* out_device);

class Decoder {
  public:
    Decoder(int backend, int device_id);
    ~Decoder();
    int Initialize();
    int GetImageInfo(const StreamParser* s, uint8_t* ncomp, int32_t* css, uint32_t* widths, uint32_t* heights, int scale_denom = 1);
    int Decode(const StreamParser* const* streams, int n, const DecodeParams& params, const DestImage* dsts);

    int Prepare(const StreamParser* const* streams, int n, const DecodeParams& params, const DestImage* dsts);
    int Run();
    int CopyCoefficients(int image, int16_t* host_out, size_t count);
    int CopyPlanes(int image, uint8_t* host_out, size_t count);
    int CopySegment(int image, uint32_t segment, uint8_t* host_out, size_t capacity, uint32_t* nbytes);
    int GetScanStatus(int image, ScanStatus* out);
    void SetProfiling(int level) { profiling_ = level; }
    const BatchStats& stats() const { return stats_; }
    const std::string& last_error() const { return err_; }
    int device_id() const { return device_id_; }
    int num_devices() const { return 1 + int(peers_.size()); }

  private:
// ... 32 lines not shown
```

### rocjpeg_b200/csrc/device_types.h

```cpp
#pragma once
#include <stdint.h>

#ifndef __CUDACC__
#ifndef __host__
#define __host__
#define __device__
#endif
#endif

namespace rjb {

constexpr int kMaxBlocksPerMcu = 10;
constexpr int kFastBits = 9;
constexpr int kFastSize = 1 << kFastBits;
constexpr int kSubCap = 1024;

enum Css : int32_t { CSS_444 = 0, CSS_440 = 1, CSS_422 = 2, CSS_420 = 3, CSS_411 = 4, CSS_400 = 5, CSS_UNKNOWN = -1 };
enum Fmt : int32_t { FMT_NATIVE = 0, FMT_YUV_PLANAR = 1, FMT_Y = 2, FMT_RGB = 3, FMT_RGB_PLANAR = 4 };

constexpr int kHuffIds = 4;
constexpr int kHuffTabs = 2 * kHuffIds;

struct HuffLutSet {
    uint32_t fast[kHuffTabs][kFastSize];
    uint32_t sub[kSubCap];
    uint32_t sub_used;
    uint32_t pad_[3];
    uint32_t upper[kHuffTabs][17];
    int32_t valoff[kHuffTabs][17];
    uint8_t vals[kHuffTabs][256];
};

struct ImageDesc {
    int32_t width, height, ncomp, css;
    int32_t mcus_x, mcus_y, bpm, restart_interval;
    int32_t total_mcus;
    int32_t hs[3], vs[3];
    int32_t blocks_w[3], blocks_h[3];
    int32_t comp_first_blk[3];
    uint8_t mcu_comp[kMaxBlocksPerMcu];
    uint8_t mcu_dc[kMaxBlocksPerMcu];
    uint8_t mcu_ac[kMaxBlocksPerMcu];
    uint8_t mcu_pair[kMaxBlocksPerMcu];
    uint8_t npairs;
    uint8_t pair_dc[3], pair_ac[3];
    uint8_t pad_[3];
    int32_t lut_set;
    int32_t qt_index[3];
    uint64_t raw_off;
    uint32_t raw_skip;
    uint32_t raw_len;
    uint32_t k0_tile0;
    uint32_t seg_keep_lo, seg_keep_hi;
    uint64_t data_off;
    uint32_t seg0, nseg;
    uint32_t sub0, nsub;
    uint64_t blk0;
    uint64_t ent0;
    uint32_t ent_cap;
    uint32_t nblocks;
    uint32_t dc_tile0;
    uint32_t comp_bits;
    uint64_t plane_off[3];
    uint32_t plane_pitch[3];
};

__host__ __device__ inline uint64_t SegmentStart(uint32_t r, uint32_t k, uint32_t S) {
    return (uint64_t(r) + uint64_t(S + 14u) * k + (S - 1u)) / S * S;
}
__host__ __device__ inline uint64_t CleanCapacity(uint32_t raw_len, uint32_t nseg, uint32_t S) {
    return (SegmentStart(raw_len, nseg, S) + S + 127u) / 128u * 128u;
}

struct ScanStatus {
    uint32_t segments_seen;
    uint32_t scan_size;
    uint32_t flags;
    uint32_t reserved;
};
constexpr uint32_t kScanNoEoi = 1u,
                   kScanStrayMarker = 2u,
                   kScanExtraRestarts = 4u,
                   kScanMissingIntervals = 8u,
                   kScanEmptyInterval = 16u,
                   kDecodeShort = 32u;
constexpr uint32_t kStatusTruncatedMask = kScanMissingIntervals | kScanEmptyInterval | kDecodeShort;

struct SegmentDesc {
    uint64_t data_off;
    uint32_t nbytes;
    uint32_t sub0;
    uint32_t blk_first;
    uint32_t blk_count;
};

struct OutputDesc {
    uint8_t* dst[4];
    uint32_t dst_pitch[4];
    int32_t x0, y0, w, h;
    int32_t fmt;
    uint32_t tile0;
    uint32_t tiles_x, tiles_y;
    int32_t direct;
    int32_t fused;
};

struct FusedImage {
    uint64_t ent0, blk0;
    uint8_t* dst[3];
    uint32_t dpitch;
    uint32_t ent_cap;
    int32_t width, height, css, fmt;
    int32_t ncomp, bpm, mcus_x, vmax;
    int32_t mpt;
    uint32_t tiles_x;
    uint32_t tile0;
    int32_t sx, sy;
    uint8_t H[3], V[3], first_blk[3], hshift[3];
    uint32_t qidx[3];
    uint32_t pitch[3], base[3];
    uint32_t comp_info[3];
};

}
```

### rocjpeg_b200/csrc/k1_huffman.cu

```cuda
#include <cuda_runtime.h>

#include <cstddef>

#include "huff_core.cuh"
#include "stages.h"

namespace rjb {

namespace {

constexpr int T = kK1Threads;
constexpr uint32_t kNoState = 0xFFFFFFFFu;

__device__ __forceinline__ uint32_t UpperIndex(const uint32_t* a, uint32_t n, uint32_t v) {
    uint32_t lo = 0, hi = n;
    while (hi - lo > 1) {
        uint32_t mid = (lo + hi) >> 1;
        if (__ldg(a + mid) <= v) lo = mid; else hi = mid;
    }
    return lo;
}

template <int CAP>
__device__ __forceinline__ uint32_t ImageOfCta(const K1Args& a, uint32_t* scratch, uint32_t cta) {
    const uint32_t n = uint32_t(a.nimages);
    if (n > uint32_t(CAP)) return UpperIndex(a.img_cta0, n, cta);
    for (uint32_t i = threadIdx.x; i < n; i += blockDim.x) scratch[i] = __ldg(a.img_cta0 + i);
    __syncthreads();
    uint32_t lo = 0, hi = n;
    while (hi - lo > 1) {
        const uint32_t mid = (lo + hi) >> 1;
        if (scratch[mid] <= cta) lo = mid; else hi = mid;
    }
    __syncthreads();
    return lo;
}

__device__ __forceinline__ uint32_t SharedAddr(const void* p) { return uint32_t(__cvta_generic_to_shared(p)); }
__device__ __forceinline__ uint32_t Lds32(uint32_t a) {
    uint32_t v;
    asm volatile("ld.shared.u32 %0, [%1];" : "=r"(v) : "r"(a));
    return v;
}
__device__ __forceinline__ uint32_t Lds16(uint32_t a) {
    uint32_t v;
    asm volatile("ld.shared.u16 %0, [%1];" : "=r"(v) : "r"(a));
    return v;
}

constexpr uint32_t kAccStop = 1u << 10;
constexpr uint32_t kAccBlockEnd = 1u << 27;
constexpr uint32_t kAccKeep = 0x001FFFFFu;
constexpr uint32_t kAccZMask = 63u << 21;

struct LutView {
    uint32_t fast_sa;
    uint32_t sub_sa;
    const HuffLutSet* set;
    const uint8_t* pair_tab;
};

__device__ __forceinline__ uint32_t CanonicalSearch(const LutView& lv, uint32_t off, uint32_t win) {
    return SlowEntry(lv.set, lv.pair_tab[(off - lv.fast_sa) >> 11], win >> 16);
}
__device__ __forceinline__ uint32_t ResolveLink(const LutView& lv, uint32_t e, uint32_t off, uint32_t win) {
    const uint32_t x = LinkBits(e);
    if (x == 0) return CanonicalSearch(lv, off, win);
    return Lds32(lv.sub_sa + ((LinkFirst(e) + ((win << kFastBits) >> (32u - x))) << 2));
}

struct Lane {
    uint32_t acc;
    uint32_t w0, w1, w2, wp;
    uint32_t sp0, sp;
    uint32_t next_dc;
    uint32_t off;

    __device__ __forceinline__ void Init(uint32_t slot_sa, uint32_t sched_sa, uint32_t key, uint32_t end_bit) {
        const uint32_t p = StateOverflow(key), end32 = (end_bit + 31u) & ~31u;
        acc = (p + 1024u - end32) | (uint32_t(StateZ(key)) << 21);
        wp = slot_sa + ((p >> 5) << 2);
        w0 = Lds32(wp);
        w1 = Lds32(wp + 4);
        w2 = Lds32(wp + 8);
        wp += 8;
        sp0 = sp = sched_sa + 2u * uint32_t(StateC(key));
        off = Lds16(sp) | (StateZ(key) ? 2048u : 0u);
// ... 522 lines not shown
                ".reg .b32 sz, bits, sh, t, rs, ex, m, v, zq;\n\t"
                "shr.u32 sz, %11, 28;\n\t"
                "and.b32 bits, %11, 31;\n\t"
                "sub.u32 sh, bits, sz;\n\t"
                "shl.b32 t, %12, sh;\n\t"
                "sub.u32 rs, 32, sz;\n\t"
                "shf.r.clamp.b32 ex, t, 0, rs;\n\t"
                "bmsk.clamp.b32 m, 0, sz;\n\t"
                "setp.lt.s32 pneg, t, 0;\n\t"
                "selp.b32 m, 0, m, pneg;\n\t"
                "sub.s32 v, ex, m;\n\t"
                "and.b32 zq, %13, 0x7e00000;\n\t"
                "setp.eq.u32 pdc, zq, 0;\n\t"
                "@pdc mov.b32 %6, v;\n\t"
                "setp.ne.u32 pnz, sz, 0;\n\t"
                "shr.u32 zq, %14, 21;\n\t"
                "@pnz mov.b32 %0, %1;\n\t"
                "@pnz mov.b32 %1, %2;\n\t"
                "@pnz mov.b32 %2, %3;\n\t"
                "@pnz prmt.b32 %3, v, zq, 0x5410;\n\t"
                "@pnz add.u32 %4, %4, 1;\n\t"
                "and.b32 zq, %4, 7;\n\t"
                "setp.eq.and.u32 phalf, zq, 4, pnz;\n\t"
                "setp.eq.and.u32 pfl, zq, 0, pnz;\n\t"
                "@phalf mov.b32 %7, %0;\n\t"
                "@phalf mov.b32 %8, %1;\n\t"
                "@phalf mov.b32 %9, %2;\n\t"
                "@phalf mov.b32 %10, %3;\n\t"
                "setp.le.and.u32 pst, %4, %15, pfl;\n\t"
                "@pst st.global.v8.b32 [%5], {%7, %8, %9, %10, %0, %1, %2, %3};\n\t"
                "@pfl add.u64 %5, %5, 32;\n\t"
                "}"
                : "+r"(q0), "+r"(q1), "+r"(q2), "+r"(q3), "+r"(n), "+l"(ep), "+r"(dcv), "+r"(h0), "+r"(h1), "+r"(h2), "+r"(h3)
                : "r"(en), "r"(win), "r"(ln.acc), "r"(nxt), "r"(n_end)
                : "memory");
            ln.CommitWrite(nxt, rp, n, rp_stop, dcv, has_dc);
            if (ln.acc & kAccStop) break;
        }
    }
    if (me.last && blk0 < limit && uint32_t(rp - recs) < limit) atomicOr(&a.status[img].flags, kDecodeShort);
    if (has_dc && (ln.acc & kAccZMask) != 0 && blk0 < limit && me.end_bit != 0) rp->dc = int16_t(dcv);
    if (n & 7u) {
        for (; n & 7u; n++) {
            q0 = q1; q1 = q2; q2 = q3; q3 = kPadEntry;
            if ((n & 7u) == 3u) { h0 = q0; h1 = q1; h2 = q2; h3 = q3; }
        }
        if (n <= n_end) {
            reinterpret_cast<uint4*>(ep)[0] = make_uint4(h0, h1, h2, h3);
            reinterpret_cast<uint4*>(ep)[1] = make_uint4(q0, q1, q2, q3);
        }
        ep += 8;
    }
    for (; n < n_end; n += 8, ep += 8) {
        reinterpret_cast<uint4*>(ep)[0] = make_uint4(kPadEntry, kPadEntry, kPadEntry, kPadEntry);
        reinterpret_cast<uint4*>(ep)[1] = make_uint4(kPadEntry, kPadEntry, kPadEntry, kPadEntry);
    }
}

template <int S>
__global__ void __launch_bounds__(T) k1_write(K1Args a) {
    PdlEntry();
    extern __shared__ __align__(16) unsigned char smem_raw[];
    uint32_t* const lut = reinterpret_cast<uint32_t*>(smem_raw);
    K1Smem<S>& sm = *reinterpret_cast<K1Smem<S>*>(smem_raw + a.lut_smem_bytes);
    const int tid = threadIdx.x;
    const uint32_t cta = blockIdx.x;
    const uint32_t img = ImageOfCta<T * K1Smem<S>::kSlotStride>(a, sm.words, cta);
    const ImageDesc& im = a.images[img];
    const int H = a.halo, TO = T - H;
    const int64_t gi = int64_t(cta) * TO + tid - H;
    const uint32_t g = uint32_t(gi);
    Sub me = Locate<S>(a, im, gi, true);
    if (tid < H) me.active = false;
    const LutView lv = StageCta<S>(sm, lut, a, im, me);
    const uint32_t st = me.active ? a.state[g] : 0;
    const uint32_t my_nnz = me.active ? a.nnz[g] : 0;
    uint32_t key = 0;
    if (me.active && !me.first) key = StateKey(a.state[g - 1]);
    WriteBody<S, false>(a, sm, lv, img, im, me, st, my_nnz, key, cta);
}

template <int S>
__device__ void IntegrateDc(const K1Args& a, uint32_t* scratch, uint32_t img, uint32_t cta);

template <int S>
__global__ void __maxnreg__(46) k1_fused(K1Args a, int max_iters) {
    PdlEntry();
    extern __shared__ __align__(16) unsigned char smem_raw[];
    uint32_t* const lut = reinterpret_cast<uint32_t*>(smem_raw);
    K1Smem<S>& sm = *reinterpret_cast<K1Smem<S>*>(smem_raw + a.lut_smem_bytes);
    const int tid = threadIdx.x;
    __shared__ uint32_t s_ticket, s_img;
    if (tid == 0) s_ticket = atomicAdd(a.cta_flag + a.total_ctas, 1u);
    __syncthreads();
    const uint32_t cta = s_ticket;
    SyncOut so = SyncBody<S, true>(a, sm, lut, 0, max_iters, cta);
    if (tid == 0) s_img = so.img;
    __threadfence();
    __syncthreads();
    if (tid == 0) asm volatile("st.release.gpu.global.u32 [%0], %1;" ::"l"(a.cta_flag + cta), "r"(1u) : "memory");
    const int H = a.halo;
    const ImageDesc& im = a.images[so.img];
    if (tid == H && so.me.active && !so.me.first && cta > 0) {
        uint32_t f;
        do {
            asm volatile("ld.acquire.gpu.global.u32 %0, [%1];" : "=r"(f) : "l"(a.cta_flag + cta - 1) : "memory");
        } while (f == 0u);
        const uint32_t g = uint32_t(int64_t(cta) * (T - H));
        if (StateKey(__ldcg(a.state + g - 1)) != so.used) atomicAdd(&a.counters[0], 1u);
    }
    Sub me = so.me;
    if (tid < H) me.active = false;
    WriteBody<S, true>(a, sm, so.lv, so.img, im, me, me.active ? so.state : 0u, me.active ? so.nnz : 0u, so.used, cta);
    if (a.k1_dc) {
        const uint32_t c = *static_cast<volatile uint32_t*>(&s_ticket);
        __threadfence();
        __syncthreads();
        if (tid == 0) asm volatile("st.release.gpu.global.u32 [%0], %1;" ::"l"(a.cta_flag + c), "r"(2u) : "memory");
        IntegrateDc<S>(a, sm.scratch, *static_cast<volatile uint32_t*>(&s_img), c);
    }
}


__device__ __forceinline__ int RecDc(const BlockRec& r) { return r.end == kNoEntry ? 0 : int(r.dc); }

struct McuDc {
    int d[kMaxBlocksPerMcu];
    int s0, s1, s2;
    template <int N>
    __device__ __forceinline__ void LoadN(const BlockRec* rec, int bpm, uint32_t comp_bits, bool active) {
        s0 = s1 = s2 = 0;
#pragma unroll
        for (int k = 0; k < N; k++) {
            d[k] = 0;
            if (active && k < bpm) {
                const uint2 r = *reinterpret_cast<const uint2*>(rec + k);
                d[k] = r.x == kNoEntry ? 0 : int(int16_t(r.y & 0xFFFFu));
            }
            const uint32_t comp = (comp_bits >> (2 * k)) & 3u;
            s0 += comp == 0u ? d[k] : 0;
            s1 += comp == 1u ? d[k] : 0;
            s2 += comp == 2u ? d[k] : 0;
        }
    }
    template <int N>
    __device__ __forceinline__ void StoreN(BlockRec* rec, int bpm, uint32_t comp_bits, int p0, int p1, int p2) const {
#pragma unroll
        for (int k = 0; k < N; k++) {
            const uint32_t comp = (comp_bits >> (2 * k)) & 3u;
            p0 += comp == 0u ? d[k] : 0;
            p1 += comp == 1u ? d[k] : 0;
            p2 += comp == 2u ? d[k] : 0;
            if (k < bpm) rec[k].dc = int16_t(comp == 0u ? p0 : comp == 1u ? p1 : p2);
        }
    }
    __device__ __forceinline__ void Load(const BlockRec* rec, int bpm, uint32_t comp_bits, bool active) {
        if (bpm == 1) LoadN<1>(rec, bpm, comp_bits, active);
        else if (bpm <= 4) LoadN<4>(rec, bpm, comp_bits, active);
        else if (bpm <= 6) LoadN<6>(rec, bpm, comp_bits, active);
        else LoadN<kMaxBlocksPerMcu>(rec, bpm, comp_bits, active);
    }
    __device__ __forceinline__ void Store(BlockRec* rec, int bpm, uint32_t comp_bits, int p0, int p1, int p2) const {
        if (bpm == 1) StoreN<1>(rec, bpm, comp_bits, p0, p1, p2);
        else if (bpm <= 4) StoreN<4>(rec, bpm, comp_bits, p0, p1, p2);
        else if (bpm <= 6) StoreN<6>(rec, bpm, comp_bits, p0, p1, p2);
        else StoreN<kMaxBlocksPerMcu>(rec, bpm, comp_bits, p0, p1, p2);
    }
};
__device__ __forceinline__ bool ResetAt(uint32_t m, int ri) { return ri > 0 ? (m % uint32_t(ri)) == 0u : m == 0u; }

__device__ __forceinline__ int64_t LastReset(int64_t m0, int64_t m1, int ri) {
    if (m1 <= m0) return -1;
    if (ri <= 0) return m0 == 0 ? 0 : -1;
    const int64_t last = ((m1 - 1) / ri) * ri;
    return last >= m0 ? last : -1;
}

__device__ __forceinline__ int LoadDc(const BlockRec* r) {
    const uint2 v = __ldcg(reinterpret_cast<const uint2*>(r));
    return v.x == kNoEntry ? 0 : int(int16_t(v.y & 0xFFFFu));
}

template <int S>
__device__ void IntegrateDc(const K1Args& a, uint32_t* scratch, uint32_t img, uint32_t cta) {
    const int tid = threadIdx.x, lane = tid & 31, warp = tid >> 5;
    constexpr int kW = T / 32;
    const ImageDesc& im = a.images[img];
    const uint32_t first = __ldg(a.img_cta0 + img);
    uint32_t* const dc_flag = a.cta_flag + a.total_ctas + 1;
    const int H = a.halo;
    if (tid == H || tid == T - 1) {
        const uint32_t enter = scratch[3 * kW];
        const int64_t gi = int64_t(cta) * (T - H) + tid - H;
        if (tid == H) {
            scratch[kDcPosSlot] = BlockPos(a, im, Locate<S>(a, im, gi, false), enter);
        } else {
            const uint2 part = a.cta_partial[cta];
            scratch[kDcPosSlot + 1] = BlockPos(a, im, Locate<S>(a, im, gi + 1, false), part.y + (part.x ? 0u : enter));
        }
    }
    if (tid == 0 && cta != first) {
        uint32_t f;
// ... 20 lines not shown
            s0 += comp == 0u ? d : 0;
            s1 += comp == 1u ? d : 0;
            s2 += comp == 2u ? d : 0;
            if (++k == bpm) { k = 0; m++; }
        }
    }
    int v0 = s0, v1 = s1, v2 = s2;
    uint32_t g = f;
#pragma unroll
    for (int d = 1; d < 32; d <<= 1) {
        const int p0 = __shfl_up_sync(0xFFFFFFFFu, v0, d);
        const int p1 = __shfl_up_sync(0xFFFFFFFFu, v1, d);
        const int p2 = __shfl_up_sync(0xFFFFFFFFu, v2, d);
        const uint32_t pg = __shfl_up_sync(0xFFFFFFFFu, g, d);
        if (lane >= d) {
            if (!g) { v0 += p0; v1 += p1; v2 += p2; }
            g |= pg;
        }
    }
    int* const ws = reinterpret_cast<int*>(scratch);
    int* const carry = ws + 4 * kW;
    if (lane == 31) { ws[4 * warp] = v0; ws[4 * warp + 1] = v1; ws[4 * warp + 2] = v2; ws[4 * warp + 3] = int(g); }
    __syncthreads();
    if (warp == 0) {
        int t0 = 0, t1 = 0, t2 = 0, tf = 0;
        for (int w = 0; w < kW; w++) {
            if (ws[4 * w + 3]) { t0 = ws[4 * w]; t1 = ws[4 * w + 1]; t2 = ws[4 * w + 2]; tf = 1; }
            else { t0 += ws[4 * w]; t1 += ws[4 * w + 1]; t2 += ws[4 * w + 2]; }
        }
        if (lane == 0) {
            a.cta_dc[2 * cta] = make_int4(t0, t1, t2, tf);
            __threadfence();
            asm volatile("st.release.gpu.global.u32 [%0], %1;" ::"l"(dc_flag + cta), "r"(1u) : "memory");
        }
        int c0 = 0, c1 = 0, c2 = 0;
        for (int64_t top = int64_t(cta); top > int64_t(first); top -= 32) {
            const int64_t k = top - 32 + lane;
            int4 e = make_int4(0, 0, 0, 0);
            uint32_t fl = 0;
            if (k >= int64_t(first)) {
                do {
                    asm volatile("ld.acquire.gpu.global.u32 %0, [%1];" : "=r"(fl) : "l"(dc_flag + k) : "memory");
                } while (fl == 0u);
                e = __ldcg(a.cta_dc + 2 * k + (fl == 2u ? 1 : 0));
            }
            const uint32_t stop = __ballot_sync(0xFFFFFFFFu, fl == 2u || e.w != 0);
            const int from = stop ? 31 - __clz(stop) : 0;
            if (lane >= from) { c0 += e.x; c1 += e.y; c2 += e.z; }
            if (stop) break;
        }
#pragma unroll
        for (int d = 16; d > 0; d >>= 1) {
            c0 += __shfl_xor_sync(0xFFFFFFFFu, c0, d);
            c1 += __shfl_xor_sync(0xFFFFFFFFu, c1, d);
            c2 += __shfl_xor_sync(0xFFFFFFFFu, c2, d);
        }
        if (lane == 0) {
            carry[0] = c0; carry[1] = c1; carry[2] = c2;
            a.cta_dc[2 * cta + 1] = tf ? make_int4(t0, t1, t2, 0) : make_int4(c0 + t0, c1 + t1, c2 + t2, 0);
            __threadfence();
            asm volatile("st.release.gpu.global.u32 [%0], %1;" ::"l"(dc_flag + cta), "r"(2u) : "memory");
        }
    }
    __syncthreads();
    int p0 = __shfl_up_sync(0xFFFFFFFFu, v0, 1), p1 = __shfl_up_sync(0xFFFFFFFFu, v1, 1), p2 = __shfl_up_sync(0xFFFFFFFFu, v2, 1);
    uint32_t open = !__shfl_up_sync(0xFFFFFFFFu, g, 1);
    if (lane == 0) { p0 = p1 = p2 = 0; open = 1; }
    for (int w = warp - 1; w >= 0 && open; w--) {
        p0 += ws[4 * w]; p1 += ws[4 * w + 1]; p2 += ws[4 * w + 2];
        if (ws[4 * w + 3]) open = 0;
    }
    if (open) { p0 += carry[0]; p1 += carry[1]; p2 += carry[2]; }
    uint32_t m = b0 / bpm, k = b0 - m * bpm;
    for (uint32_t b = b0; b < b1; b++) {
        if (k == 0 && ResetAt(m, ri)) p0 = p1 = p2 = 0;
        const int d = LoadDc(rec + b);
        const uint32_t comp = (comp_bits >> (2 * k)) & 3u;
        p0 += comp == 0u ? d : 0;
        p1 += comp == 1u ? d : 0;
        p2 += comp == 2u ? d : 0;
        rec[b].dc = int16_t(comp == 0u ? p0 : comp == 1u ? p1 : p2);
        if (++k == bpm) { k = 0; m++; }
    }
}

__global__ void __launch_bounds__(kDcTileMcus) dc_sums(K1Args a) {
    PdlEntry();
    __shared__ int red[3];
    const int tid = threadIdx.x;
    const uint32_t tile = blockIdx.x;
    const uint32_t img = UpperIndex(a.img_dctile0, uint32_t(a.nimages), tile);
    const ImageDesc& im = a.images[img];
    const int64_t m0 = int64_t(tile - a.img_dctile0[img]) * kDcTileMcus;
    const int64_t m1 = min(m0 + kDcTileMcus, int64_t(im.total_mcus));
    const int64_t reset = LastReset(m0, m1, im.restart_interval);
    const int64_t m = m0 + tid;
    if (tid < 3) red[tid] = 0;
    __syncthreads();
    McuDc mcu;
    mcu.Load(a.blk_rec + im.blk0 + m * im.bpm, im.bpm, im.comp_bits, m < m1 && m >= reset);
    const int s[3] = {mcu.s0, mcu.s1, mcu.s2};
#pragma unroll
    for (int c = 0; c < 3; c++) {
        int v = s[c];
#pragma unroll
        for (int d = 16; d > 0; d >>= 1) v += __shfl_xor_sync(0xFFFFFFFFu, v, d);
        if ((tid & 31) == 0 && v) atomicAdd(&red[c], v);
    }
    __syncthreads();
    if (tid == 0) a.dc_partial[tile] = make_int3(red[0], red[1], red[2]);
}

__global__ void __launch_bounds__(kScanThreads) dc_scan(K1Args a) {
    PdlEntry();
    __shared__ int s_v[kScanThreads / 32][3];
    __shared__ uint32_t s_f[kScanThreads / 32];
    const uint32_t img = blockIdx.x;
    const int tid = threadIdx.x, lane = tid & 31, warp = tid >> 5;
    const ImageDesc& im = a.images[img];
    const uint32_t t0 = a.img_dctile0[img], t1 = a.img_dctile0[img + 1];
    const int ri = im.restart_interval;
    int c0 = 0, c1 = 0, c2 = 0;
    for (uint32_t base = t0; base < t1; base += kScanThreads) {
        const uint32_t k = base + tid;
        int3 part = make_int3(0, 0, 0);
        uint32_t f = 0;
        if (k < t1) {
            part = a.dc_partial[k];
            const int64_t m0 = int64_t(k - t0) * kDcTileMcus;
            f = LastReset(m0, min(m0 + kDcTileMcus, int64_t(im.total_mcus)), ri) >= 0 ? 1u : 0u;
        }
        int v0 = part.x, v1 = part.y, v2 = part.z;
#pragma unroll
        for (int d = 1; d < 32; d <<= 1) {
            const int p0 = __shfl_up_sync(0xFFFFFFFFu, v0, d);
            const int p1 = __shfl_up_sync(0xFFFFFFFFu, v1, d);
            const int p2 = __shfl_up_sync(0xFFFFFFFFu, v2, d);
            const uint32_t pf = __shfl_up_sync(0xFFFFFFFFu, f, d);
            if (lane >= d) {
                if (!f) { v0 += p0; v1 += p1; v2 += p2; }
                f |= pf;
            }
        }
        __syncthreads();
        if (lane == 31) { s_v[warp][0] = v0; s_v[warp][1] = v1; s_v[warp][2] = v2; s_f[warp] = f; }
        __syncthreads();
        int q0 = 0, q1 = 0, q2 = 0;
        uint32_t qf = 0;
        for (int w = 0; w < warp; w++) {
            if (s_f[w]) { q0 = s_v[w][0]; q1 = s_v[w][1]; q2 = s_v[w][2]; } else { q0 += s_v[w][0]; q1 += s_v[w][1]; q2 += s_v[w][2]; }
            qf |= s_f[w];
        }
        if (!qf) { q0 += c0; q1 += c1; q2 += c2; }
        int x0 = __shfl_up_sync(0xFFFFFFFFu, v0, 1), x1 = __shfl_up_sync(0xFFFFFFFFu, v1, 1), x2 = __shfl_up_sync(0xFFFFFFFFu, v2, 1);
        uint32_t xf = __shfl_up_sync(0xFFFFFFFFu, f, 1);
        if (lane == 0) { x0 = x1 = x2 = 0; xf = 0; }
        if (k < t1) a.dc_carry[k] = xf ? make_int3(x0, x1, x2) : make_int3(x0 + q0, x1 + q1, x2 + q2);
        int w0 = 0, w1 = 0, w2 = 0;
        uint32_t wf = 0;
        for (int w = 0; w < kScanThreads / 32; w++) {
            if (s_f[w]) { w0 = s_v[w][0]; w1 = s_v[w][1]; w2 = s_v[w][2]; } else { w0 += s_v[w][0]; w1 += s_v[w][1]; w2 += s_v[w][2]; }
            wf |= s_f[w];
        }
        if (wf) { c0 = w0; c1 = w1; c2 = w2; } else { c0 += w0; c1 += w1; c2 += w2; }
    }
}
// ... 73 lines not shown
        mcu.Load(rec, bpm, comp_bits, active);
        int v0 = mcu.s0, v1 = mcu.s1, v2 = mcu.s2;
        uint32_t f = reset_here ? 1u : 0u;
#pragma unroll
        for (int d = 1; d < 32; d <<= 1) {
            const int p0 = __shfl_up_sync(0xFFFFFFFFu, v0, d);
            const int p1 = __shfl_up_sync(0xFFFFFFFFu, v1, d);
            const int p2 = __shfl_up_sync(0xFFFFFFFFu, v2, d);
            const uint32_t pf = __shfl_up_sync(0xFFFFFFFFu, f, d);
            if (lane >= d) {
                if (!f) { v0 += p0; v1 += p1; v2 += p2; }
                f |= pf;
            }
        }
        __syncthreads();
        if (lane == 31) { wsum[warp][0] = v0; wsum[warp][1] = v1; wsum[warp][2] = v2; wflag[warp] = int(f); }
        __syncthreads();
        if (warp == 0) {
            int t0 = 0, t1 = 0, t2 = 0;
            uint32_t tf = 0;
            if (lane < kWarps) { t0 = wsum[lane][0]; t1 = wsum[lane][1]; t2 = wsum[lane][2]; tf = uint32_t(wflag[lane]); }
#pragma unroll
            for (int d = 1; d < 32; d <<= 1) {
                const int p0 = __shfl_up_sync(0xFFFFFFFFu, t0, d);
                const int p1 = __shfl_up_sync(0xFFFFFFFFu, t1, d);
                const int p2 = __shfl_up_sync(0xFFFFFFFFu, t2, d);
                const uint32_t pf = __shfl_up_sync(0xFFFFFFFFu, tf, d);
                if (lane >= d) {
                    if (!tf) { t0 += p0; t1 += p1; t2 += p2; }
                    tf |= pf;
                }
            }
            if (!tf) { t0 += c0; t1 += c1; t2 += c2; }
            int x0 = __shfl_up_sync(0xFFFFFFFFu, t0, 1), x1 = __shfl_up_sync(0xFFFFFFFFu, t1, 1), x2 = __shfl_up_sync(0xFFFFFFFFu, t2, 1);
            if (lane == 0) { x0 = c0; x1 = c1; x2 = c2; }
            if (lane < kWarps) { wpre[lane][0] = x0; wpre[lane][1] = x1; wpre[lane][2] = x2; }
            c0 = __shfl_sync(0xFFFFFFFFu, t0, 31);
            c1 = __shfl_sync(0xFFFFFFFFu, t1, 31);
            c2 = __shfl_sync(0xFFFFFFFFu, t2, 31);
        }
        __syncthreads();
        if (active) {
            const bool open = (f == 0);
            const int p0 = v0 - mcu.s0 + (open ? wpre[warp][0] : 0), p1 = v1 - mcu.s1 + (open ? wpre[warp][1] : 0),
                      p2 = v2 - mcu.s2 + (open ? wpre[warp][2] : 0);
            mcu.Store(rec, bpm, comp_bits, reset_here ? 0 : p0, reset_here ? 0 : p1, reset_here ? 0 : p2);
        }
    }
}

__global__ void k1_clear_short(K1Args a) {
    const int i = int(blockIdx.x * blockDim.x + threadIdx.x);
    if (i < a.nimages) a.status[i].flags &= ~kDecodeShort;
}

template <int S>
cudaError_t SyncImpl(const K1Args& a, int round, cudaStream_t stream, int max_iters = T + 1) {
    static_assert(S <= 128, "the packed decoder state holds bit positions below 2048");
    const size_t smem = sizeof(K1Smem<S>) + a.lut_smem_bytes;
    if (smem > 48 * 1024) return cudaErrorInvalidValue;
    if (round >= 0) return LaunchPdl(k1_sync<S>, dim3(a.total_ctas), dim3(T), smem, stream, a, round, max_iters);
    return LaunchPdl(k1_write<S>, dim3(a.total_ctas), dim3(T), smem, stream, a);
}

}

cudaError_t LaunchK1Sync(const K1Args& a, int round, cudaStream_t stream, int max_iters) {
    if (a.total_ctas == 0) return cudaSuccess;
    if (max_iters <= 0) max_iters = T + 1;
    switch (a.sub_bytes) {
        case 32: return SyncImpl<32>(a, round, stream, max_iters);
        case 64: return SyncImpl<64>(a, round, stream, max_iters);
        case 128: return SyncImpl<128>(a, round, stream, max_iters);
        default: return cudaErrorInvalidValue;
    }
}

cudaError_t LaunchK1ClearShort(const K1Args& a, cudaStream_t stream) {
    if (a.nimages <= 0) return cudaSuccess;
    k1_clear_short<<<dim3((a.nimages + 255) / 256), dim3(256), 0, stream>>>(a);
    return cudaGetLastError();
}

cudaError_t LaunchK1Fused(const K1Args& a, cudaStream_t stream) {
    if (a.total_ctas == 0) return cudaSuccess;
    const int max_iters = T + 1;
    switch (a.sub_bytes) {
        case 32: { const size_t smem = sizeof(K1Smem<32>) + a.lut_smem_bytes; if (smem > 48 * 1024) return cudaErrorInvalidValue;
                   return LaunchPdl(k1_fused<32>, dim3(a.total_ctas), dim3(T), smem, stream, a, max_iters); }
        case 64: { const size_t smem = sizeof(K1Smem<64>) + a.lut_smem_bytes; if (smem > 48 * 1024) return cudaErrorInvalidValue;
                   return LaunchPdl(k1_fused<64>, dim3(a.total_ctas), dim3(T), smem, stream, a, max_iters); }
        case 128: { const size_t smem = sizeof(K1Smem<128>) + a.lut_smem_bytes; if (smem > 48 * 1024) return cudaErrorInvalidValue;
                    return LaunchPdl(k1_fused<128>, dim3(a.total_ctas), dim3(T), smem, stream, a, max_iters); }
        default: return cudaErrorInvalidValue;
    }
}

cudaError_t LaunchK1Write(const K1Args& a, cudaStream_t stream) {
    if (a.total_ctas == 0) return cudaSuccess;
    if (!a.inline_scan) {
        const cudaError_t e = LaunchPdl(k1_scan, dim3(a.nimages), dim3(kScanThreads), 0, stream, a);
        if (e != cudaSuccess) return e;
    }
    switch (a.sub_bytes) {
        case 32: return SyncImpl<32>(a, -1, stream);
        case 64: return SyncImpl<64>(a, -1, stream);
        case 128: return SyncImpl<128>(a, -1, stream);
        default: return cudaErrorInvalidValue;
    }
}

cudaError_t LaunchDcScan(const K1Args& a, cudaStream_t stream) {
    if (a.total_dc_tiles == 0) return cudaSuccess;
    if (a.dc_image) return LaunchPdl(dc_image, dim3(a.nimages), dim3(kDcImageThreads), 0, stream, a);
    cudaError_t e = LaunchPdl(dc_sums, dim3(a.total_dc_tiles), dim3(kDcTileMcus), 0, stream, a);
    if (e == cudaSuccess) e = LaunchPdl(dc_scan, dim3(a.nimages), dim3(kScanThreads), 0, stream, a);
    if (e == cudaSuccess) e = LaunchPdl(dc_apply, dim3(a.total_dc_tiles), dim3(kDcTileMcus), 0, stream, a);
    return e;
}

cudaError_t PreloadK1() {
    cudaFuncAttributes at;
    cudaError_t e = cudaSuccess;
    if (e == cudaSuccess) e = cudaFuncGetAttributes(&at, k1_sync<128>);
    if (e == cudaSuccess) e = cudaFuncGetAttributes(&at, k1_sync<64>);
    if (e == cudaSuccess) e = cudaFuncGetAttributes(&at, k1_sync<32>);
    if (e == cudaSuccess) e = cudaFuncGetAttributes(&at, k1_write<128>);
    if (e == cudaSuccess) e = cudaFuncGetAttributes(&at, k1_write<64>);
    if (e == cudaSuccess) e = cudaFuncGetAttributes(&at, k1_write<32>);
    if (e == cudaSuccess) e = cudaFuncGetAttributes(&at, k1_fused<128>);
    if (e == cudaSuccess) e = cudaFuncGetAttributes(&at, k1_fused<64>);
    if (e == cudaSuccess) e = cudaFuncGetAttributes(&at, k1_fused<32>);
    if (e == cudaSuccess) e = cudaFuncGetAttributes(&at, k1_scan);
    if (e == cudaSuccess) e = cudaFuncGetAttributes(&at, dc_sums);
    if (e == cudaSuccess) e = cudaFuncGetAttributes(&at, dc_scan);
    if (e == cudaSuccess) e = cudaFuncGetAttributes(&at, dc_apply);
    if (e == cudaSuccess) e = cudaFuncGetAttributes(&at, dc_image);
    return e;
}

}
```

### rocjpeg_b200/csrc/k23_fused.cu

```cuda
#include <cuda_runtime.h>

#include "idct_core.cuh"
#include "k3_rows.cuh"
#include "stages.h"

namespace rjb {
namespace {

using namespace idct;
using namespace k3;

constexpr int kStripW = 256;
constexpr int kFThreads = 256;
constexpr int kMaxBlocks = 128;
constexpr int kLumaBytes = 16 * kStripW, kChromaBytes = 8 * kStripW;
static_assert(kStripW == kTileW, "the row routines assume 8 samples per lane over the strip");

__device__ __forceinline__ uint32_t SharedU32(const void* p) {
    uint32_t a = uint32_t(__cvta_generic_to_shared(p));
    asm volatile("mov.u32 %0, %0;" : "+r"(a));
    return a;
}
__device__ __forceinline__ uint32_t Lds32(uint32_t a) {
    uint32_t v;
    asm volatile("ld.shared.u32 %0, [%1];" : "=r"(v) : "r"(a));
    return v;
}
__device__ __forceinline__ uint4 Lds128(uint32_t a) {
    uint4 v;
    asm volatile("ld.shared.v4.u32 {%0, %1, %2, %3}, [%4];" : "=r"(v.x), "=r"(v.y), "=r"(v.z), "=r"(v.w) : "r"(a));
    return v;
}
__device__ __forceinline__ void Sts32(uint32_t a, uint32_t v) { asm volatile("st.shared.u32 [%0], %1;" ::"r"(a), "r"(v) : "memory"); }
__device__ __forceinline__ void Sts64(uint32_t a, uint32_t x, uint32_t y) { asm volatile("st.shared.v2.u32 [%0], {%1, %2};" ::"r"(a), "r"(x), "r"(y) : "memory"); }
__device__ __forceinline__ void Sts128(uint32_t a, uint4 v) {
    asm volatile("st.shared.v4.u32 [%0], {%1, %2, %3, %4};" ::"r"(a), "r"(v.x), "r"(v.y), "r"(v.z), "r"(v.w) : "memory");
}

__global__ void __launch_bounds__(kFThreads, 6) k23_fused(K23Args a) {
    PdlEntry();
    constexpr int kRS = 12, kBS = 104;
    __shared__ __align__(16) int ws[32 * kBS];
    __shared__ __align__(16) uint8_t s_pl[kLumaBytes + 2 * kChromaBytes];
    __shared__ __align__(16) uint8_t s_buf[kFThreads / 32][kRowBuf];
    __shared__ uint32_t s_tab[3][64];
    __shared__ __align__(16) uint4 s_meta[kMaxBlocks];
    __shared__ K3Job s_job;
    const int tid = threadIdx.x, lane = tid & 31, warp = tid >> 5;
    const FusedImage& fi = a.fused[__ldg(a.tile_img + blockIdx.x) & 0xFFFFu];
    const uint32_t t = blockIdx.x - fi.tile0;
    const int mrow = int(t / fi.tiles_x), tx = int(t - uint32_t(mrow) * fi.tiles_x);
    const int m0 = tx * fi.mpt, nm = min(fi.mpt, fi.mcus_x - m0);
    const int ncomp = fi.ncomp;
    const int nbw0 = nm * fi.H[0], nbw1 = ncomp > 1 ? nm * fi.H[1] : 0, nbw2 = ncomp > 2 ? nm * fi.H[2] : 0;
    const int cnt0 = nbw0 * fi.V[0], cnt1 = nbw1 * (ncomp > 1 ? fi.V[1] : 0), cnt2 = nbw2 * (ncomp > 2 ? fi.V[2] : 0);
    const int nblocks = cnt0 + cnt1 + cnt2;
    const uint32_t* entries = a.entries + fi.ent0;
    const BlockRec* rec = a.blk_rec + fi.blk0;
    const int xt = tx * kStripW, rows = 8 * fi.vmax, y0t = mrow * rows;
    if (tid == 0) {
        K3Job j;
        for (int c = 0; c < 3; c++) {
            const int cc = c < ncomp ? c : 0;
            const int shx = cc ? fi.sx : 0, shy = cc ? fi.sy : 0;
            j.pitch[c] = fi.pitch[cc];
            j.p[c] = s_pl + fi.base[cc] - (size_t(y0t >> shy) * fi.pitch[cc] + size_t(xt >> shx));
            j.dst[c] = fi.dst[c];
            j.dpitch[c] = fi.dpitch;
        }
        j.dst[3] = nullptr;
        j.dpitch[3] = 0;
        j.W = fi.width; j.H = fi.height; j.x0 = 0; j.y0 = 0; j.css = fi.css; j.fmt = fi.fmt;
        j.xt = xt;
        j.ty = mrow;
        j.nx = min(kStripW, fi.width - xt);
        s_job = j;
    }
    for (int idx = tid; idx < ncomp * 64; idx += kFThreads) {
        const int c = idx >> 6, code = idx & 63;
        const int nat = kZigzag[(code + 63) & 63];
        s_tab[c][code] = uint32_t(code == 1 ? 8 * 4 : ((nat >> 3) * kRS + (nat & 7)) * 4) | (uint32_t(__ldg(a.qtables + size_t(fi.qidx[c]) * 64 + nat)) << 16);
    }
    if (tid < kMaxBlocks) {
        uint4 m = make_uint4(0u, 0u, 0u, 0u);
        if (tid < nblocks) {
            int g = tid, c = 0, nbw = nbw0;
            if (g >= cnt0) { g -= cnt0; c = 1; nbw = nbw1; if (g >= cnt1) { g -= cnt1; c = 2; nbw = nbw2; } }
            const int v = g / nbw, bx = g - v * nbw;
            const int H = fi.H[c];
            const size_t blk = size_t(mrow * fi.mcus_x + m0 + (bx >> fi.hshift[c])) * size_t(fi.bpm) + size_t(fi.first_blk[c] + v * H + (bx & (H - 1)));
            const uint2 r = __ldg(reinterpret_cast<const uint2*>(rec + blk));
            uint32_t e0 = blk ? __ldg(&rec[blk - 1].end) : 0u, e1 = r.x;
            if (e0 == kNoEntry || e1 == kNoEntry || e1 < e0 || e1 - e0 > 0xFFFFu || e1 > fi.ent_cap) e1 = e0 = 0;
            m.x = e0;
            m.y = (e1 - e0) | (uint32_t(c) << 16) | (1u << 24);
            m.z = uint32_t(int(int16_t(r.y & 0xFFFFu)) * int(__ldg(a.qtables + size_t(fi.qidx[c]) * 64)));
            m.w = (fi.base[c] + uint32_t(v * 8) * fi.pitch[c] + uint32_t(bx * 8)) | (fi.pitch[c] << 16);
        }
        s_meta[tid] = m;
    }
    __syncthreads();
    const int b = tid >> 3, jj = tid & 7;
    const uint32_t my_sa = SharedU32(ws) + uint32_t(b * kBS * 4);
    const uint32_t row_sa = my_sa + uint32_t(jj * kRS * 4), col_sa = my_sa + uint32_t(jj * 4);
    const uint32_t tab_sa0 = SharedU32(&s_tab[0][0]), pl_sa = SharedU32(s_pl);
    uint32_t meta_sa = SharedU32(s_meta) + uint32_t(b * 16);
    const uint32_t* const ent_j = entries + jj;
    const uint32_t meta_end = SharedU32(s_meta) + uint32_t(nblocks * 16);
#pragma unroll 1
    for (; meta_sa < meta_end + uint32_t(b * 16); meta_sa += 32 * 16) {
        const uint4 m = Lds128(meta_sa);
        const uint32_t n = m.y & 0xFFFFu;
        const uint32_t* ep = ent_j + m.x;
        const uint32_t k = uint32_t(jj);
        uint32_t e[4];
#pragma unroll
        for (int u = 0; u < 4; u++) e[u] = (k + 8u * u < n) ? __ldg(ep + 8 * u) : 0u;
        Sts128(row_sa, make_uint4(jj == 0 ? m.z : 0u, 0u, 0u, 0u));
        Sts128(row_sa + 16, make_uint4(0u, 0u, 0u, 0u));
        __syncwarp();
        const uint32_t tab_sa = tab_sa0 + ((m.y >> 8) & 0x300u);
        auto put = [&](uint32_t en) {
            const uint32_t t = Lds32(tab_sa + ((en >> 14) & 0xFCu));
            Sts32(my_sa + (t & 0xFFFFu), uint32_t(int(int16_t(en & 0xFFFFu)) * int(t >> 16)));
        };
#pragma unroll
        for (int u = 0; u < 4; u++)
            if (k + 8u * u < n) put(e[u]);
        for (uint32_t kk = k + 32u; kk < n; kk += 8) put(__ldg(ep + (kk - k)));
        __syncwarp();
        int in[8], out[8];
#pragma unroll
        for (int r = 0; r < 8; r++) in[r] = int(Lds32(col_sa + uint32_t(r * kRS * 4)));
        Islow8<11>(in, out, 1 << 10);
#pragma unroll
        for (int r = 0; r < 8; r++) Sts32(col_sa + uint32_t(r * kRS * 4), uint32_t(out[r]));
        __syncwarp();
        {
            const uint4 lo = Lds128(row_sa), hi = Lds128(row_sa + 16);
            in[0] = int(lo.x); in[1] = int(lo.y); in[2] = int(lo.z); in[3] = int(lo.w);
            in[4] = int(hi.x); in[5] = int(hi.y); in[6] = int(hi.z); in[7] = int(hi.w);
            Islow8<18>(in, out, (1 << 17) + (128 << 18));
            if (m.y >> 24) Sts64(pl_sa + (m.w & 0xFFFFu) + uint32_t(jj) * (m.w >> 16), PackSat4(out[0], out[1], out[2], out[3]), PackSat4(out[4], out[5], out[6], out[7]));
        }
        __syncwarp();
    }
    __syncthreads();
    const K3Job& j = s_job;
    const int fmt = j.fmt, css = j.css;
    if (j.nx <= 0) return;
    if (fmt == FMT_RGB && (j.dst[0] == nullptr || j.dpitch[0] == 0)) return;
    if (fmt == FMT_RGB_PLANAR && (!j.dst[0] || !j.dst[1] || !j.dst[2] || j.dpitch[0] == 0)) return;
    const int sx = css == CSS_411 ? 2 : (css == CSS_422 || css == CSS_420) ? 1 : 0;
    const int sy = (css == CSS_440 || css == CSS_420) ? 1 : 0;
    const bool gray = (css == CSS_400);
    const uintptr_t bases = fmt == FMT_RGB ? reinterpret_cast<uintptr_t>(j.dst[0]) + size_t(j.xt) * 3
                                           : (reinterpret_cast<uintptr_t>(j.dst[0]) | reinterpret_cast<uintptr_t>(j.dst[1]) |
                                              reinterpret_cast<uintptr_t>(j.dst[2])) + size_t(j.xt);
    uint8_t* buf = s_buf[warp];
    for (int r = warp; r < rows; r += kFThreads / 32) {
        const int y = y0t + r;
        if (y >= j.H) break;
        const bool dst_ok = ((bases | (size_t(y) * j.dpitch[0])) & 3) == 0;
        if (dst_ok) {
            if (sx == 2) RowRgbFast<2, true>(j, sy, gray, y, lane); else if (sx) RowRgbFast<1, true>(j, sy, gray, y, lane); else RowRgbFast<0, true>(j, sy, gray, y, lane);
        } else {
            if (sx == 2) RowRgbStaged<2, true>(j, sy, gray, buf, y, lane); else if (sx) RowRgbStaged<1, true>(j, sy, gray, buf, y, lane);
            else RowRgbStaged<0, true>(j, sy, gray, buf, y, lane);
        }
    }
}


constexpr int kWarpW = 32;
constexpr int kWarpBlocks = 16;
constexpr int kWarpLuma = kWarpW * 16, kWarpChroma = 256;

struct __align__(16) WarpSmem {
    int ws[4 * 104];
    uint4 meta[kWarpBlocks];
    uint8_t pl[kWarpLuma + 2 * kWarpChroma];
};

__global__ void __launch_bounds__(kFThreads, 6) k23_warp(K23Args a) {
    PdlEntry();
    constexpr int kRS = 12, kBS = 104;
    __shared__ WarpSmem s_w[kFThreads / 32];
    __shared__ uint32_t s_tab[3][64];
    const int tid = threadIdx.x, lane = tid & 31, warp = tid >> 5;
    const uint32_t tile = __ldg(a.tile_img_w + blockIdx.x);
    const FusedImage& gfi = a.fused[tile & 0xFFFFu];
    __shared__ __align__(16) FusedImage s_fi;
    static_assert(sizeof(FusedImage) % 16 == 0, "copied as 16-byte vectors");
    if (tid < int(sizeof(FusedImage) / 16)) reinterpret_cast<uint4*>(&s_fi)[tid] = __ldg(reinterpret_cast<const uint4*>(&gfi) + tid);
    {
        const int ncomp_g = gfi.ncomp;
        for (int idx = tid; idx < ncomp_g * 64; idx += kFThreads) {
            const int c = idx >> 6, code = idx & 63;
            const int nat = kZigzag[(code + 63) & 63];
            s_tab[c][code] = uint32_t(code == 1 ? 8 * 4 : ((nat >> 3) * kRS + (nat & 7)) * 4) | (uint32_t(__ldg(a.qtables + size_t(gfi.qidx[c]) * 64 + nat)) << 16);
        }
    }
    __syncthreads();
    const FusedImage& fi = s_fi;
    const int mrow = int(tile >> 16), tx = int(blockIdx.x - fi.tile0) - mrow * int(fi.tiles_x);
    const int ncomp = fi.ncomp;
    const int mpt = fi.mpt, mcus_x = fi.mcus_x;
    const int mpw = mpt >> 3;
    const int m0 = tx * mpt + warp * mpw, nm = min(mpw, mcus_x - m0);
    if (nm <= 0) return;
    WarpSmem& sw = s_w[warp];
    int nblocks;
    {
        const uint32_t ci0 = fi.comp_info[0], ci1 = ncomp > 1 ? fi.comp_info[1] : 0u, ci2 = ncomp > 2 ? fi.comp_info[2] : 0u;
        const int nbw0 = nm * int(ci0 & 0xFFu), nbw1 = nm * int(ci1 & 0xFFu), nbw2 = nm * int(ci2 & 0xFFu);
        const int cnt0 = nbw0 * int((ci0 >> 8) & 0xFFu), cnt1 = nbw1 * int((ci1 >> 8) & 0xFFu), cnt2 = nbw2 * int((ci2 >> 8) & 0xFFu);
        nblocks = cnt0 + cnt1 + cnt2;
        if (lane < kWarpBlocks) {
            uint4 m = make_uint4(0u, 0u, 0u, 0u);
            if (lane < nblocks) {
                int g = lane, c = 0, nbw = nbw0;
                uint32_t ci = ci0;
                if (g >= cnt0) { g -= cnt0; c = 1; nbw = nbw1; ci = ci1; if (g >= cnt1) { g -= cnt1; c = 2; nbw = nbw2; ci = ci2; } }
                const int v = g >= nbw ? 1 : 0, bx = g - (v ? nbw : 0);
                const uint32_t H = ci & 0xFFu;
                const uint32_t blk = uint32_t(mrow * mcus_x + m0 + (bx >> (ci >> 24))) * uint32_t(fi.bpm) + ((ci >> 16) & 0xFFu) + uint32_t(v) * H + (uint32_t(bx) & (H - 1u));
                const BlockRec* rp = a.blk_rec + fi.blk0 + blk;
                const uint2 r = __ldg(reinterpret_cast<const uint2*>(rp));
                uint32_t e0 = blk ? __ldg(&rp[-1].end) : 0u, e1 = r.x;
                if (e0 == kNoEntry || e1 == kNoEntry || e1 < e0 || e1 - e0 > 0xFFFFu || e1 > fi.ent_cap) e1 = e0 = 0;
                const uint32_t pitch = uint32_t(8 * mpw) * H;
                const uint32_t base = c == 0 ? 0u : uint32_t(kWarpLuma + (c - 1) * kWarpChroma);
                m.x = e0;
                m.y = (e1 - e0) | (uint32_t(c) << 16) | (1u << 24);
                m.z = uint32_t(int(int16_t(r.y & 0xFFFFu)) * int(s_tab[c][1] >> 16));
                m.w = (base + uint32_t(v * 8) * pitch + uint32_t(bx * 8)) | (pitch << 16);
            }
            sw.meta[lane] = m;
        }
    }
    __syncwarp();
    {
        const int b = lane >> 3, jj = lane & 7;
        const uint32_t my_sa = SharedU32(sw.ws) + uint32_t(b * kBS * 4);
        const uint32_t row_sa = my_sa + uint32_t(jj * kRS * 4), col_sa = my_sa + uint32_t(jj * 4);
        const uint32_t tab_sa0 = SharedU32(&s_tab[0][0]), pl_sa = SharedU32(sw.pl);
        uint32_t meta_sa = SharedU32(sw.meta) + uint32_t(b * 16);
        const uint32_t* const ent_j = a.entries + fi.ent0 + jj;
        const uint32_t meta_end = meta_sa + uint32_t(nblocks * 16);
#pragma unroll 1
        for (; meta_sa < meta_end; meta_sa += 4 * 16) {
            const uint4 m = Lds128(meta_sa);
            const uint32_t n = m.y & 0xFFFFu;
            const uint32_t* ep = ent_j + m.x;
            const uint32_t k = uint32_t(jj);
            uint32_t e[4];
#pragma unroll
            for (int u = 0; u < 4; u++) e[u] = (k + 8u * u < n) ? __ldg(ep + 8 * u) : 0u;
            Sts128(row_sa, make_uint4(jj == 0 ? m.z : 0u, 0u, 0u, 0u));
            Sts128(row_sa + 16, make_uint4(0u, 0u, 0u, 0u));
            __syncwarp();
            const uint32_t tab_sa = tab_sa0 + ((m.y >> 8) & 0x300u);
            auto put = [&](uint32_t en) {
                const uint32_t tt = Lds32(tab_sa + ((en >> 14) & 0xFCu));
                Sts32(my_sa + (tt & 0xFFFFu), uint32_t(int(int16_t(en & 0xFFFFu)) * int(tt >> 16)));
            };
#pragma unroll
            for (int u = 0; u < 4; u++)
                if (k + 8u * u < n) put(e[u]);
            for (uint32_t kk = k + 32u; kk < n; kk += 8) put(__ldg(ep + (kk - k)));
            __syncwarp();
            int in[8], out[8];
#pragma unroll
            for (int r = 0; r < 8; r++) in[r] = int(Lds32(col_sa + uint32_t(r * kRS * 4)));
            Islow8<11>(in, out, 1 << 10);
#pragma unroll
            for (int r = 0; r < 8; r++) Sts32(col_sa + uint32_t(r * kRS * 4), uint32_t(out[r]));
            __syncwarp();
            {
                const uint4 lo = Lds128(row_sa), hi = Lds128(row_sa + 16);
                in[0] = int(lo.x); in[1] = int(lo.y); in[2] = int(lo.z); in[3] = int(lo.w);
                in[4] = int(hi.x); in[5] = int(hi.y); in[6] = int(hi.z); in[7] = int(hi.w);
                Islow8<18>(in, out, (1 << 17) + (128 << 18));
                if (m.y >> 24) Sts64(pl_sa + (m.w & 0xFFFFu) + uint32_t(jj) * (m.w >> 16), PackSat4(out[0], out[1], out[2], out[3]), PackSat4(out[4], out[5], out[6], out[7]));
            }
            __syncwarp();
        }
    }
    const int fmt = fi.fmt;
    uint8_t* const d0 = fi.dst[0];
    uint8_t* const d1 = fi.dst[1];
    uint8_t* const d2 = fi.dst[2];
    const uint32_t dpitch = fi.dpitch;
    if (d0 == nullptr || dpitch == 0) return;
    if (fmt == FMT_RGB_PLANAR && (!d1 || !d2)) return;
    const bool gray = fi.css == CSS_400;
    const int sx = fi.sx, sy = fi.sy;
    const int rows = 8 * fi.vmax, y0 = mrow * rows;
    const int seg = lane & 3, x = tx * kStripW + warp * kWarpW + seg * 8;
    const int n = fi.width - x;
    if (n <= 0) return;
    const uint32_t pl_sa = SharedU32(sw.pl);
    const uint32_t cp = ncomp > 1 ? uint32_t(8 * mpw * fi.H[1]) : 0u;
    for (int r = lane >> 2; r < rows; r += 8) {
        const int y = y0 + r;
        if (y >= fi.height) break;
        uint2 yy;
        asm volatile("ld.shared.v2.u32 {%0, %1}, [%2];" : "=r"(yy.x), "=r"(yy.y) : "r"(pl_sa + uint32_t(r * kWarpW + seg * 8)));
        Rgb8 o;
        if (gray) {
            o.r = o.g = o.b = yy;
        } else {
            const uint32_t ca = pl_sa + uint32_t(kWarpLuma) + uint32_t(r >> sy) * cp + uint32_t((seg * 8) >> sx);
            uint2 uu = make_uint2(0u, 0u), vv = make_uint2(0u, 0u);
            if (sx == 0) {
                asm volatile("ld.shared.v2.u32 {%0, %1}, [%2];" : "=r"(uu.x), "=r"(uu.y) : "r"(ca));
                asm volatile("ld.shared.v2.u32 {%0, %1}, [%2];" : "=r"(vv.x), "=r"(vv.y) : "r"(ca + uint32_t(kWarpChroma)));
                o = Convert8<0>(yy, uu, vv);
            } else if (sx == 1) {
                uu.x = Lds32(ca);
                vv.x = Lds32(ca + uint32_t(kWarpChroma));
                o = Convert8<1>(yy, uu, vv);
            } else {
                asm volatile("ld.shared.u16 %0, [%1];" : "=r"(uu.x) : "r"(ca));
                asm volatile("ld.shared.u16 %0, [%1];" : "=r"(vv.x) : "r"(ca + uint32_t(kWarpChroma)));
                o = Convert8<2>(yy, uu, vv);
            }
        }
        StoreRgb8(fmt, d0, d1, d2, dpitch, y, x, n, o);
    }
}

}

cudaError_t LaunchK23Fused(const K23Args& a, cudaStream_t stream) {
    cudaError_t e = cudaSuccess;
    if (a.total_tiles_w != 0) e = LaunchPdl(k23_warp, dim3(a.total_tiles_w), dim3(kFThreads), 0, stream, a);
    if (e == cudaSuccess && a.total_tiles != 0) e = LaunchPdl(k23_fused, dim3(a.total_tiles), dim3(kFThreads), 0, stream, a);
    return e;
}

cudaError_t PreloadK23() {
    cudaFuncAttributes at;
    cudaError_t e = cudaFuncGetAttributes(&at, k23_fused);
    if (e == cudaSuccess) e = cudaFuncGetAttributes(&at, k23_warp);
    return e;
}

}
```

### rocjpeg_b200/csrc/stages.h

```cpp
#pragma once
#include <cuda_runtime.h>
#include <stdint.h>

#include "device_types.h"

namespace rjb {

#ifdef __CUDACC__
#ifndef RJB_PDL_TRIGGER
#define RJB_PDL_TRIGGER 0
#endif
__device__ __forceinline__ void PdlEntry() {
#if RJB_PDL_TRIGGER
    asm volatile("griddepcontrol.launch_dependents;");
#endif
    asm volatile("griddepcontrol.wait;" ::: "memory");
}

template <class... KArgs, class... Args>
inline cudaError_t LaunchPdl(void (*kernel)(KArgs...), dim3 grid, dim3 block, size_t smem, cudaStream_t stream, Args... args) {
    cudaLaunchConfig_t cfg = {};
    cfg.gridDim = grid;
    cfg.blockDim = block;
    cfg.dynamicSmemBytes = smem;
// ... 1 lines not shown
    cudaLaunchAttribute attr[1];
    attr[0].id = cudaLaunchAttributeProgrammaticStreamSerialization;
    attr[0].val.programmaticStreamSerializationAllowed = 1;
    cfg.attrs = attr;
    cfg.numAttrs = 1;
    return cudaLaunchKernelEx(&cfg, kernel, KArgs(args)...);
}
#endif

constexpr int kK0TileBytes = 16384;
constexpr int kK1Threads = 128;
constexpr int kDcImageMaxMcus = 4096;
constexpr int kDcTileMcus = 256;
constexpr int kMaxSyncRounds = 8;
constexpr int kK3TileW = 256;
constexpr int kK3TileH = 32;
constexpr uint32_t kNoEntry = 0xFFFFFFFFu;

struct BlockRec {
    uint32_t end;
    int16_t dc;
    int16_t pad_;
};

struct K0Args {
    const ImageDesc* images;
    SegmentDesc* segments;
    const uint32_t* img_tile0;
    const uint8_t* raw;
    uint8_t* clean;
    uint4* tile_sum;
    uint4* tile_carry;
    ScanStatus* status;
    int nimages;
    uint32_t total_tiles;
    int sub_bytes;
    int inline_scan;
};
struct GatherItem {
    const uint8_t* src;
    uint64_t dst_off;
    uint32_t nbytes;
    uint32_t pad_;
};
cudaError_t LaunchK0Reduce(const K0Args& a, cudaStream_t stream);
cudaError_t LaunchGatherReduce(const K0Args& a, const GatherItem* items, cudaStream_t stream);
cudaError_t LaunchK0Destuff(const K0Args& a, cudaStream_t stream);
cudaError_t PreloadK0();

struct K1Args {
    const ImageDesc* images;
    const SegmentDesc* segments;
    const uint32_t* img_cta0;
    const uint32_t* img_dctile0;
    const uint8_t* scan;
    const HuffLutSet* luts;
    uint32_t* state;
    uint32_t* used;
    uint32_t* sub_seg;
    uint32_t* nnz;
    uint2* cta_partial;
    uint32_t* cta_entries;
    uint2* cta_carry;
    uint32_t* cta_flag;
    int4* cta_dc;
    int3* dc_partial;
    int3* dc_carry;
    uint32_t* counters;
    uint32_t* counters_next;
    ScanStatus* status;
    uint32_t* entries;
    BlockRec* blk_rec;
    int nimages;
    uint32_t total_ctas;
    uint32_t total_dc_tiles;
    int sub_bytes;
    uint32_t lut_smem_bytes;
    uint32_t rec_fill_vecs;
    int halo;
    int inline_scan;
    int fusable;
    int dc_image;
    int k1_dc;
};

cudaError_t LaunchK1Sync(const K1Args& a, int round, cudaStream_t stream, int max_iters = 0);
cudaError_t LaunchK1Write(const K1Args& a, cudaStream_t stream);
cudaError_t LaunchK1Fused(const K1Args& a, cudaStream_t stream);
cudaError_t LaunchK1ClearShort(const K1Args& a, cudaStream_t stream);
cudaError_t LaunchDcScan(const K1Args& a, cudaStream_t stream);

struct K2Args {
    const ImageDesc* images;
    const OutputDesc* outputs;
    int force_planes;
    const uint32_t* img_tile0;
    const uint16_t* qtables;
    const uint32_t* entries;
    const BlockRec* blk_rec;
    uint8_t* planes;
    int nimages;
    uint32_t total_tiles;
};
cudaError_t LaunchK2Idct(const K2Args& a, cudaStream_t stream);
cudaError_t LaunchK2Scaled(const K2Args& a, int scale_denom, cudaStream_t stream);

struct K23Args {
    const FusedImage* fused;
    const uint32_t* tile_img;
    const uint32_t* tile_img_w;
    const uint16_t* qtables;
    const uint32_t* entries;
    const BlockRec* blk_rec;
    int nimages;
    uint32_t total_tiles, total_tiles_w;
};
cudaError_t LaunchK23Fused(const K23Args& a, cudaStream_t stream);
cudaError_t PreloadK23();

struct K3Args {
    const ImageDesc* images;
    const OutputDesc* outputs;
    const uint32_t* img_tile0;
    const uint8_t* planes;
    int nimages;
    uint32_t total_tiles;
};
cudaError_t LaunchK3Output(const K3Args& a, cudaStream_t stream);

cudaError_t PreloadK1();
cudaError_t PreloadK2();
cudaError_t PreloadK2Scaled();
cudaError_t PreloadK3();

}
```

Baseline: 110,800.

## Run fused IDCT+colour work early inside Huffman kernel for finished pictures

CTAs of the fused Huffman kernel finish their per-picture DC integration, count completed CTAs per picture, and push pictures whose CTAs have all finished onto a ready queue. Idle warps then claim IDCT/colour units from that queue through a per-picture atomic cursor, until a fraction of the grid is done. The later k23_warp kernel skips units already claimed and can exit tiles early. The aim is to overlap the IDCT/output stage with the Huffman tail. In exchange it adds atomics, coherent loads and shared-memory reuse, and risks contention or load imbalance.

```diff
diff --git a/include/rocjpeg_b200_ext.h b/include/rocjpeg_b200_ext.h
--- a/include/rocjpeg_b200_ext.h
+++ b/include/rocjpeg_b200_ext.h
@@ -33,6 +33,8 @@
     uint32_t truncated_images;
     uint32_t pad_;
     uint64_t fused_blocks;
+    uint32_t early_units;
+    uint32_t pad2_;
 } RocJpegB200Stats;
 
 RocJpegStatus rocJpegB200SetProfiling(RocJpegHandle handle, int enable);
diff --git a/rocjpeg_b200/api.py b/rocjpeg_b200/api.py
--- a/rocjpeg_b200/api.py
+++ b/rocjpeg_b200/api.py
@@ -48,6 +48,7 @@
         ("subsequence_bytes", C.c_int32), ("lanes", C.c_int32),
         ("host_submit_ms", C.c_float), ("host_wait_ms", C.c_float), ("devices", C.c_int32),
         ("entries", C.c_uint64), ("truncated_images", C.c_uint32), ("pad_", C.c_uint32), ("fused_blocks", C.c_uint64),
+        ("early_units", C.c_uint32), ("pad2_", C.c_uint32),
     ]
 
 
diff --git a/rocjpeg_b200/csrc/api.cpp b/rocjpeg_b200/csrc/api.cpp
--- a/rocjpeg_b200/csrc/api.cpp
+++ b/rocjpeg_b200/csrc/api.cpp
@@ -265,6 +265,7 @@
     stats->entries = s.entries;
     stats->truncated_images = s.truncated_images;
     stats->fused_blocks = s.fused_blocks;
+    stats->early_units = s.early_units;
     return ROCJPEG_STATUS_SUCCESS;
 }
 
diff --git a/rocjpeg_b200/csrc/decoder.cpp b/rocjpeg_b200/csrc/decoder.cpp
--- a/rocjpeg_b200/csrc/decoder.cpp
+++ b/rocjpeg_b200/csrc/decoder.cpp
@@ -604,6 +604,7 @@
         any_direct_ = any_direct_ || od.direct || od.fused || !whole;
         needs_planes_ = needs_planes_ || tiles;
         k2_needed_ = k2_needed_ || (!od.fused && d == 1);
+        im.fused_w = -1;
         if (od.fused) {
             FusedImage fi = {};
             fi.ent0 = im.ent0; fi.blk0 = im.blk0; fi.ent_cap = im.ent_cap;
@@ -634,6 +635,8 @@
                 off += c == 0 ? 16u * kK3TileW : 8u * kK3TileW;
             }
             const uint32_t ntiles = fi.tiles_x * uint32_t(p.mcus_y);
+            fi.units = ntiles * uint32_t(kK3TileW / 32);
+            if (aligned) im.fused_w = int32_t(h_fused_.size());
             std::vector<uint32_t>& list = aligned ? h_tile_img_w_ : h_tile_img_;
             for (uint32_t r = 0; r < uint32_t(p.mcus_y); r++) list.insert(list.end(), fi.tiles_x, uint32_t(h_fused_.size()) | (r << 16));
             h_fused_.push_back(fi);
@@ -759,7 +762,7 @@
                  o_tile_carry = carve(size_t(k0_.total_tiles) * 16), o_status = carve(n * sizeof(ScanStatus)), o_entries = carve(entry_count_ * 4),
                  o_blkrec = carve(coef_blocks_ * sizeof(BlockRec)), o_nnz = carve(nsub_total_ * 4), o_state = carve(nsub_total_ * 4),
                  o_used = carve(nsub_total_ * 4), o_subseg = carve(nsub_total_ * 4), o_cta_entries = carve(size_t(k1_.total_ctas) * 4),
-                 o_cta_partial = carve(size_t(k1_.total_ctas) * 8), o_cta_carry = carve(size_t(k1_.total_ctas) * 8), o_cta_flag = carve(size_t(k1_.total_ctas) * 8 + 4),
+                 o_cta_partial = carve(size_t(k1_.total_ctas) * 8), o_cta_carry = carve(size_t(k1_.total_ctas) * 8), o_cta_flag = carve(CtaFlagBytes() + EarlyK23Bytes()),
                  o_cta_dc = carve(size_t(k1_.total_ctas) * 32),
                  o_dc_partial = carve(size_t(k1_.total_dc_tiles) * 12), o_dc_carry = carve(size_t(k1_.total_dc_tiles) * 12),
                  o_end = carve(0);
@@ -793,6 +796,11 @@
     k1_.dc_carry = reinterpret_cast<int3*>(base + o_dc_carry);
     k1_.cta_carry = reinterpret_cast<uint2*>(base + o_cta_carry);
     k1_.cta_flag = reinterpret_cast<uint32_t*>(base + o_cta_flag);
+    k1_.pic_done = reinterpret_cast<uint32_t*>(base + o_cta_flag + CtaFlagBytes());
+    k1_.ready = k1_.pic_done + n + 2;
+    k1_.cursor = k1_.ready + 1 + h_fused_.size();
+    k1_.fused = reinterpret_cast<const FusedImage*>(d + L.fused);
+    k1_.qtables = reinterpret_cast<const uint16_t*>(d + L.qtables);
     k1_.cta_dc = reinterpret_cast<int4*>(base + o_cta_dc);
     k1_.entries = reinterpret_cast<uint32_t*>(base + o_entries);
     k1_.blk_rec = reinterpret_cast<BlockRec*>(base + o_blkrec);
@@ -822,6 +830,7 @@
     k23_.qtables = k2_.qtables;
     k23_.entries = k1_.entries;
     k23_.blk_rec = k1_.blk_rec;
+    k23_.cursor = k1_.cursor;
 
     guard.Acquire();
     host_ms_[1] = NowMs();
@@ -897,7 +906,14 @@
     const bool k1_fuse_ok = EnvInt("ROCJPEG_B200_NO_K1_FUSE", 0) == 0 && std::getenv("ROCJPEG_B200_SYNC_ROUNDS") == nullptr;
     const bool k1_fused = k1_fuse_ok && k1_.fusable && k1_.total_ctas != 0;
     k1_.k1_dc = k1_fused && k1_.dc_image && EnvInt("ROCJPEG_B200_NO_K1_DC", 0) == 0 ? 1 : 0;
-    if (k1_fused) RJB_CUDA(cudaMemsetAsync(k1_.cta_flag, 0, size_t(k1_.total_ctas) * 8 + 4, stream_));
+    bool any_warp_picture = false;
+    for (const ImageDesc& im : h_images_) any_warp_picture = any_warp_picture || im.fused_w >= 0;
+    k1_.early_k23 = k1_.k1_dc && any_warp_picture && EarlyK23Fits(k1_) && EnvInt("ROCJPEG_B200_NO_EARLY_K23", 0) == 0 ? 1 : 0;
+    k23_.claim = k1_.early_k23;
+    k1_.early_warps = EnvInt("RJB_X_WARPS", 4);
+    k1_.early_stop = EnvInt("RJB_X_STOP", 8);
+    k23_.precheck = EnvInt("RJB_X_PRE", 1);
+    if (k1_fused) RJB_CUDA(cudaMemsetAsync(k1_.cta_flag, 0, CtaFlagBytes() + (k1_.early_k23 ? EarlyK23Bytes() : 0), stream_));
     if (!(include_upload && tiles_reduced_)) {
         RJB_CUDA(LaunchK0Reduce(k0_, stream_));
         stats_.kernel_launches++;
@@ -981,7 +997,9 @@
         uint32_t idct_launches = 0;
         const int st = LaunchIdct(false, &idct_launches);
         if (st != kSuccess) return st;
-        RJB_CUDA(LaunchK23Fused(k23_, stream_));
+        K23Args k23 = k23_;
+        k23.claim = 0;
+        RJB_CUDA(LaunchK23Fused(k23, stream_));
         RJB_CUDA(LaunchK3Output(k3_, stream_));
         RJB_CUDA(cudaMemcpyAsync(h_counters_.data(), k1_.counters, 256, cudaMemcpyDeviceToHost, stream_));
         RJB_CUDA(cudaMemcpyAsync(h_counters_.data() + 256, k0_.status, h_images_.size() * sizeof(ScanStatus), cudaMemcpyDeviceToHost, stream_));
@@ -989,6 +1007,7 @@
         stats_.kernel_launches += 8;
     }
     stats_.entries = cnt[2 * kMaxSyncRounds];
+    stats_.early_units = cnt[2 * kMaxSyncRounds + 1];
     ScanStatus* st = reinterpret_cast<ScanStatus*>(h_counters_.data() + 256);
     truncated_images_ = 0;
     for (size_t i = 0; i < h_images_.size(); i++) {
@@ -1161,6 +1180,7 @@
         stats_.subsequences += s.subsequences;
         stats_.plane_bytes += s.plane_bytes;
         stats_.fused_blocks += s.fused_blocks;
+        stats_.early_units += s.early_units;
         stats_.output_bytes += s.output_bytes;
         stats_.h2d_bytes += s.h2d_bytes;
         stats_.d2h_bytes += s.d2h_bytes;
@@ -1289,6 +1309,7 @@
         total.subsequences += s.subsequences;
         total.plane_bytes += s.plane_bytes;
         total.fused_blocks += s.fused_blocks;
+        total.early_units += s.early_units;
         total.output_bytes += s.output_bytes;
         total.h2d_bytes += s.h2d_bytes;
         total.d2h_bytes += s.d2h_bytes;
diff --git a/rocjpeg_b200/csrc/decoder.h b/rocjpeg_b200/csrc/decoder.h
--- a/rocjpeg_b200/csrc/decoder.h
+++ b/rocjpeg_b200/csrc/decoder.h
@@ -75,6 +75,7 @@
     float host_submit_ms = 0, host_wait_ms = 0;
     int devices = 1;
     uint32_t truncated_images = 0;
+    uint32_t early_units = 0;
 };
 
 class SubmitPool {
@@ -130,6 +131,8 @@
 
   private:
     struct Layout;
+    size_t CtaFlagBytes() const { return size_t(k1_.total_ctas) * 8 + 4; }
+    size_t EarlyK23Bytes() const { return (h_images_.size() + 3 + 2 * h_fused_.size()) * 4; }
     int Fail(int status, const std::string& why);
     int LaunchIdct(bool force_planes, uint32_t* launches);
 
diff --git a/rocjpeg_b200/csrc/device_types.h b/rocjpeg_b200/csrc/device_types.h
--- a/rocjpeg_b200/csrc/device_types.h
+++ b/rocjpeg_b200/csrc/device_types.h
@@ -63,6 +63,7 @@
     uint32_t comp_bits;
     uint64_t plane_off[3];
     uint32_t plane_pitch[3];
+    int32_t fused_w;
 };
 
 __host__ __device__ inline uint64_t SegmentStart(uint32_t r, uint32_t k, uint32_t S) {
@@ -120,6 +121,8 @@
     uint32_t qidx[3];
     uint32_t pitch[3], base[3];
     uint32_t comp_info[3];
+    uint32_t units;
+    uint32_t pad_[3];
 };
 
 }
diff --git a/rocjpeg_b200/csrc/k1_huffman.cu b/rocjpeg_b200/csrc/k1_huffman.cu
--- a/rocjpeg_b200/csrc/k1_huffman.cu
+++ b/rocjpeg_b200/csrc/k1_huffman.cu
@@ -3,6 +3,7 @@
 #include <cstddef>
 
 #include "huff_core.cuh"
+#include "k23_warp.cuh"
 #include "stages.h"
 
 namespace rjb {
@@ -691,6 +692,7 @@
 
 template <int S>
 __device__ void IntegrateDc(const K1Args& a, uint32_t* scratch, uint32_t img, uint32_t cta);
+__device__ __forceinline__ void EarlyK23(const K1Args& a, unsigned char* smem, uint32_t img);
 
 template <int S>
 __global__ void __maxnreg__(46) k1_fused(K1Args a, int max_iters) {
@@ -727,6 +729,7 @@
         __syncthreads();
         if (tid == 0) asm volatile("st.release.gpu.global.u32 [%0], %1;" ::"l"(a.cta_flag + c), "r"(2u) : "memory");
         IntegrateDc<S>(a, sm.scratch, *static_cast<volatile uint32_t*>(&s_img), c);
+        if (a.early_k23) EarlyK23(a, smem_raw, *static_cast<volatile uint32_t*>(&s_img));
     }
 }
 
@@ -913,6 +916,87 @@
         rec[b].dc = int16_t(comp == 0u ? p0 : comp == 1u ? p1 : p2);
         if (++k == bpm) { k = 0; m++; }
     }
+}
+
+struct __align__(16) EarlySmem {
+    k23w::WarpSmem w;
+    uint32_t tab[3 * 64];
+    FusedImage fi;
+    uint32_t scan, have, converted, pad_;
+};
+constexpr size_t kEarlySmemBytes = size_t(T / 32) * sizeof(EarlySmem);
+
+__device__ __forceinline__ uint32_t LdRelaxed(const uint32_t* p) {
+    uint32_t v;
+    asm volatile("ld.relaxed.gpu.global.u32 %0, [%1];" : "=r"(v) : "l"(p) : "memory");
+    return v;
+}
+
+__device__ __forceinline__ void EarlyK23(const K1Args& a, unsigned char* smem, uint32_t img) {
+    const int tid = threadIdx.x, lane = tid & 31, warp = tid >> 5;
+    uint32_t* const grid_done = a.pic_done + a.nimages;
+    uint32_t* const ready_head = a.pic_done + a.nimages + 1;
+    __threadfence();
+    __syncthreads();
+    if (tid == 0) {
+        const int p = a.images[img].fused_w;
+        if (p >= 0) {
+            const uint32_t ctas = __ldg(a.img_cta0 + img + 1) - __ldg(a.img_cta0 + img);
+            uint32_t old;
+            asm volatile("atom.acq_rel.gpu.global.add.u32 %0, [%1], 1;" : "=r"(old) : "l"(a.pic_done + img) : "memory");
+            if (old + 1 == ctas) {
+                const uint32_t slot = atomicAdd(a.ready, 1u);
+                asm volatile("st.release.gpu.global.u32 [%0], %1;" ::"l"(a.ready + 1 + slot), "r"(uint32_t(p) + 1u) : "memory");
+            }
+        }
+        asm volatile("red.release.gpu.global.add.u32 [%0], 1;" ::"l"(grid_done) : "memory");
+    }
+    if (warp >= a.early_warps) return;
+    if (*reinterpret_cast<volatile const uint32_t*>(a.cta_flag + a.total_ctas) < a.total_ctas) return;
+    const uint32_t stop_at = uint32_t((uint64_t(a.total_ctas) * uint32_t(a.early_stop)) >> 3);
+    EarlySmem& es = reinterpret_cast<EarlySmem*>(smem)[warp];
+    volatile uint32_t& scan = es.scan;
+    volatile uint32_t& have = es.have;
+    volatile uint32_t& converted = es.converted;
+    if (lane == 0) { scan = 0; have = ~0u; converted = 0; }
+    __syncwarp();
+    for (;;) {
+        uint32_t u = ~0u, p = 0;
+        if (lane == 0) {
+            uint32_t s = max(uint32_t(scan), LdRelaxed(ready_head));
+            while (LdRelaxed(grid_done) < stop_at && s < LdRelaxed(a.ready)) {
+                const uint32_t q = LdRelaxed(a.ready + 1 + s);
+                if (q == 0u) break;
+                const uint32_t units = __ldg(&a.fused[q - 1u].units);
+                if (LdRelaxed(a.cursor + (q - 1u)) < units) {
+                    const uint32_t v = atomicAdd(a.cursor + (q - 1u), 1u);
+                    if (v < units) { u = v; p = q - 1u; break; }
+                }
+                s++;
+                atomicMax(ready_head, s);
+            }
+            scan = s;
+            if (u != ~0u && p != have) asm volatile("fence.acq_rel.gpu;" ::: "memory");
+        }
+        u = __shfl_sync(0xFFFFFFFFu, u, 0);
+        if (u == ~0u) break;
+        p = __shfl_sync(0xFFFFFFFFu, p, 0);
+        if (p != have) {
+            if (lane < int(sizeof(FusedImage) / 16))
+                reinterpret_cast<uint4*>(&es.fi)[lane] = __ldg(reinterpret_cast<const uint4*>(a.fused + p) + lane);
+            __syncwarp();
+            for (int idx = lane; idx < es.fi.ncomp * 64; idx += 32) es.tab[idx] = k23w::TableWord(a.qtables, es.fi.qidx[idx >> 6], idx & 63);
+            __syncwarp();
+            if (lane == 0) have = p;
+        }
+        __syncwarp();
+        const uint32_t t = u / uint32_t(k23w::kWarpsPerStrip);
+        const uint32_t mrow = t / es.fi.tiles_x;
+        k23w::WarpUnit<true>(es.fi, es.tab, es.w, a.entries, a.blk_rec, int(mrow), int(t - mrow * es.fi.tiles_x), int(u % uint32_t(k23w::kWarpsPerStrip)), lane);
+        __syncwarp();
+        if (lane == 0) converted = converted + 1;
+    }
+    if (lane == 0 && converted) atomicAdd(&a.counters[2 * kMaxSyncRounds + 1], converted);
 }
 
 __global__ void __launch_bounds__(kDcTileMcus) dc_sums(K1Args a) {
@@ -1152,6 +1236,11 @@
     return cudaGetLastError();
 }
 
+bool EarlyK23Fits(const K1Args& a) {
+    const size_t stage = a.sub_bytes == 32 ? sizeof(K1Smem<32>) : a.sub_bytes == 64 ? sizeof(K1Smem<64>) : sizeof(K1Smem<128>);
+    return stage + a.lut_smem_bytes >= kEarlySmemBytes;
+}
+
 cudaError_t LaunchK1Fused(const K1Args& a, cudaStream_t stream) {
     if (a.total_ctas == 0) return cudaSuccess;
     const int max_iters = T + 1;
diff --git a/rocjpeg_b200/csrc/k23_fused.cu b/rocjpeg_b200/csrc/k23_fused.cu
--- a/rocjpeg_b200/csrc/k23_fused.cu
+++ b/rocjpeg_b200/csrc/k23_fused.cu
@@ -1,6 +1,7 @@
 #include <cuda_runtime.h>
 
 #include "idct_core.cuh"
+#include "k23_warp.cuh"
 #include "k3_rows.cuh"
 #include "stages.h"
 
@@ -9,37 +10,15 @@
 
 using namespace idct;
 using namespace k3;
-
-constexpr int kStripW = 256;
+using namespace k23w;
+
 constexpr int kFThreads = 256;
 constexpr int kMaxBlocks = 128;
 constexpr int kLumaBytes = 16 * kStripW, kChromaBytes = 8 * kStripW;
 static_assert(kStripW == kTileW, "the row routines assume 8 samples per lane over the strip");
 
-__device__ __forceinline__ uint32_t SharedU32(const void* p) {
-    uint32_t a = uint32_t(__cvta_generic_to_shared(p));
-    asm volatile("mov.u32 %0, %0;" : "+r"(a));
-    return a;
-}
-__device__ __forceinline__ uint32_t Lds32(uint32_t a) {
-    uint32_t v;
-    asm volatile("ld.shared.u32 %0, [%1];" : "=r"(v) : "r"(a));
-    return v;
-}
-__device__ __forceinline__ uint4 Lds128(uint32_t a) {
-    uint4 v;
-    asm volatile("ld.shared.v4.u32 {%0, %1, %2, %3}, [%4];" : "=r"(v.x), "=r"(v.y), "=r"(v.z), "=r"(v.w) : "r"(a));
-    return v;
-}
-__device__ __forceinline__ void Sts32(uint32_t a, uint32_t v) { asm volatile("st.shared.u32 [%0], %1;" ::"r"(a), "r"(v) : "memory"); }
-__device__ __forceinline__ void Sts64(uint32_t a, uint32_t x, uint32_t y) { asm volatile("st.shared.v2.u32 [%0], {%1, %2};" ::"r"(a), "r"(x), "r"(y) : "memory"); }
-__device__ __forceinline__ void Sts128(uint32_t a, uint4 v) {
-    asm volatile("st.shared.v4.u32 [%0], {%1, %2, %3, %4};" ::"r"(a), "r"(v.x), "r"(v.y), "r"(v.z), "r"(v.w) : "memory");
-}
-
 __global__ void __launch_bounds__(kFThreads, 6) k23_fused(K23Args a) {
     PdlEntry();
-    constexpr int kRS = 12, kBS = 104;
     __shared__ __align__(16) int ws[32 * kBS];
     __shared__ __align__(16) uint8_t s_pl[kLumaBytes + 2 * kChromaBytes];
     __shared__ __align__(16) uint8_t s_buf[kFThreads / 32][kRowBuf];
@@ -172,163 +151,40 @@
 }
 
 
-constexpr int kWarpW = 32;
-constexpr int kWarpBlocks = 16;
-constexpr int kWarpLuma = kWarpW * 16, kWarpChroma = 256;
-
-struct __align__(16) WarpSmem {
-    int ws[4 * 104];
-    uint4 meta[kWarpBlocks];
-    uint8_t pl[kWarpLuma + 2 * kWarpChroma];
-};
-
 __global__ void __launch_bounds__(kFThreads, 6) k23_warp(K23Args a) {
     PdlEntry();
-    constexpr int kRS = 12, kBS = 104;
     __shared__ WarpSmem s_w[kFThreads / 32];
     __shared__ uint32_t s_tab[3][64];
     const int tid = threadIdx.x, lane = tid & 31, warp = tid >> 5;
     const uint32_t tile = __ldg(a.tile_img_w + blockIdx.x);
     const FusedImage& gfi = a.fused[tile & 0xFFFFu];
+    if (a.claim && a.precheck) {
+        __shared__ uint32_t s_left;
+        if (tid == 0) s_left = __ldcg(a.cursor + (tile & 0xFFFFu)) < __ldg(&gfi.units) ? 1u : 0u;
+        __syncthreads();
+        if (!s_left) return;
+    }
     __shared__ __align__(16) FusedImage s_fi;
     static_assert(sizeof(FusedImage) % 16 == 0, "copied as 16-byte vectors");
     if (tid < int(sizeof(FusedImage) / 16)) reinterpret_cast<uint4*>(&s_fi)[tid] = __ldg(reinterpret_cast<const uint4*>(&gfi) + tid);
     {
         const int ncomp_g = gfi.ncomp;
-        for (int idx = tid; idx < ncomp_g * 64; idx += kFThreads) {
-            const int c = idx >> 6, code = idx & 63;
-            const int nat = kZigzag[(code + 63) & 63];
-            s_tab[c][code] = uint32_t(code == 1 ? 8 * 4 : ((nat >> 3) * kRS + (nat & 7)) * 4) | (uint32_t(__ldg(a.qtables + size_t(gfi.qidx[c]) * 64 + nat)) << 16);
-        }
+        for (int idx = tid; idx < ncomp_g * 64; idx += kFThreads) s_tab[idx >> 6][idx & 63] = TableWord(a.qtables, gfi.qidx[idx >> 6], idx & 63);
     }
     __syncthreads();
     const FusedImage& fi = s_fi;
-    const int mrow = int(tile >> 16), tx = int(blockIdx.x - fi.tile0) - mrow * int(fi.tiles_x);
-    const int ncomp = fi.ncomp;
-    const int mpt = fi.mpt, mcus_x = fi.mcus_x;
-    const int mpw = mpt >> 3;
-    const int m0 = tx * mpt + warp * mpw, nm = min(mpw, mcus_x - m0);
-    if (nm <= 0) return;
-    WarpSmem& sw = s_w[warp];
-    int nblocks;
-    {
-        const uint32_t ci0 = fi.comp_info[0], ci1 = ncomp > 1 ? fi.comp_info[1] : 0u, ci2 = ncomp > 2 ? fi.comp_info[2] : 0u;
-        const int nbw0 = nm * int(ci0 & 0xFFu), nbw1 = nm * int(ci1 & 0xFFu), nbw2 = nm * int(ci2 & 0xFFu);
-        const int cnt0 = nbw0 * int((ci0 >> 8) & 0xFFu), cnt1 = nbw1 * int((ci1 >> 8) & 0xFFu), cnt2 = nbw2 * int((ci2 >> 8) & 0xFFu);
-        nblocks = cnt0 + cnt1 + cnt2;
-        if (lane < kWarpBlocks) {
-            uint4 m = make_uint4(0u, 0u, 0u, 0u);
-            if (lane < nblocks) {
-                int g = lane, c = 0, nbw = nbw0;
-                uint32_t ci = ci0;
-                if (g >= cnt0) { g -= cnt0; c = 1; nbw = nbw1; ci = ci1; if (g >= cnt1) { g -= cnt1; c = 2; nbw = nbw2; ci = ci2; } }
-                const int v = g >= nbw ? 1 : 0, bx = g - (v ? nbw : 0);
-                const uint32_t H = ci & 0xFFu;
-                const uint32_t blk = uint32_t(mrow * mcus_x + m0 + (bx >> (ci >> 24))) * uint32_t(fi.bpm) + ((ci >> 16) & 0xFFu) + uint32_t(v) * H + (uint32_t(bx) & (H - 1u));
-                const BlockRec* rp = a.blk_rec + fi.blk0 + blk;
-                const uint2 r = __ldg(reinterpret_cast<const uint2*>(rp));
-                uint32_t e0 = blk ? __ldg(&rp[-1].end) : 0u, e1 = r.x;
-                if (e0 == kNoEntry || e1 == kNoEntry || e1 < e0 || e1 - e0 > 0xFFFFu || e1 > fi.ent_cap) e1 = e0 = 0;
-                const uint32_t pitch = uint32_t(8 * mpw) * H;
-                const uint32_t base = c == 0 ? 0u : uint32_t(kWarpLuma + (c - 1) * kWarpChroma);
-                m.x = e0;
-                m.y = (e1 - e0) | (uint32_t(c) << 16) | (1u << 24);
-                m.z = uint32_t(int(int16_t(r.y & 0xFFFFu)) * int(s_tab[c][1] >> 16));
-                m.w = (base + uint32_t(v * 8) * pitch + uint32_t(bx * 8)) | (pitch << 16);
-            }
-            sw.meta[lane] = m;
-        }
-    }
-    __syncwarp();
-    {
-        const int b = lane >> 3, jj = lane & 7;
-        const uint32_t my_sa = SharedU32(sw.ws) + uint32_t(b * kBS * 4);
-        const uint32_t row_sa = my_sa + uint32_t(jj * kRS * 4), col_sa = my_sa + uint32_t(jj * 4);
-        const uint32_t tab_sa0 = SharedU32(&s_tab[0][0]), pl_sa = SharedU32(sw.pl);
-        uint32_t meta_sa = SharedU32(sw.meta) + uint32_t(b * 16);
-        const uint32_t* const ent_j = a.entries + fi.ent0 + jj;
-        const uint32_t meta_end = meta_sa + uint32_t(nblocks * 16);
-#pragma unroll 1
-        for (; meta_sa < meta_end; meta_sa += 4 * 16) {
-            const uint4 m = Lds128(meta_sa);
-            const uint32_t n = m.y & 0xFFFFu;
-            const uint32_t* ep = ent_j + m.x;
-            const uint32_t k = uint32_t(jj);
-            uint32_t e[4];
-#pragma unroll
-            for (int u = 0; u < 4; u++) e[u] = (k + 8u * u < n) ? __ldg(ep + 8 * u) : 0u;
-            Sts128(row_sa, make_uint4(jj == 0 ? m.z : 0u, 0u, 0u, 0u));
-            Sts128(row_sa + 16, make_uint4(0u, 0u, 0u, 0u));
-            __syncwarp();
-            const uint32_t tab_sa = tab_sa0 + ((m.y >> 8) & 0x300u);
-            auto put = [&](uint32_t en) {
-                const uint32_t tt = Lds32(tab_sa + ((en >> 14) & 0xFCu));
-                Sts32(my_sa + (tt & 0xFFFFu), uint32_t(int(int16_t(en & 0xFFFFu)) * int(tt >> 16)));
-            };
-#pragma unroll
-            for (int u = 0; u < 4; u++)
-                if (k + 8u * u < n) put(e[u]);
-            for (uint32_t kk = k + 32u; kk < n; kk += 8) put(__ldg(ep + (kk - k)));
-            __syncwarp();
-            int in[8], out[8];
-#pragma unroll
-            for (int r = 0; r < 8; r++) in[r] = int(Lds32(col_sa + uint32_t(r * kRS * 4)));
-            Islow8<11>(in, out, 1 << 10);
-#pragma unroll
-            for (int r = 0; r < 8; r++) Sts32(col_sa + uint32_t(r * kRS * 4), uint32_t(out[r]));
-            __syncwarp();
-            {
-                const uint4 lo = Lds128(row_sa), hi = Lds128(row_sa + 16);
-                in[0] = int(lo.x); in[1] = int(lo.y); in[2] = int(lo.z); in[3] = int(lo.w);
-                in[4] = int(hi.x); in[5] = int(hi.y); in[6] = int(hi.z); in[7] = int(hi.w);
-                Islow8<18>(in, out, (1 << 17) + (128 << 18));
-                if (m.y >> 24) Sts64(pl_sa + (m.w & 0xFFFFu) + uint32_t(jj) * (m.w >> 16), PackSat4(out[0], out[1], out[2], out[3]), PackSat4(out[4], out[5], out[6], out[7]));
-            }
-            __syncwarp();
-        }
-    }
-    const int fmt = fi.fmt;
-    uint8_t* const d0 = fi.dst[0];
-    uint8_t* const d1 = fi.dst[1];
-    uint8_t* const d2 = fi.dst[2];
-    const uint32_t dpitch = fi.dpitch;
-    if (d0 == nullptr || dpitch == 0) return;
-    if (fmt == FMT_RGB_PLANAR && (!d1 || !d2)) return;
-    const bool gray = fi.css == CSS_400;
-    const int sx = fi.sx, sy = fi.sy;
-    const int rows = 8 * fi.vmax, y0 = mrow * rows;
-    const int seg = lane & 3, x = tx * kStripW + warp * kWarpW + seg * 8;
-    const int n = fi.width - x;
-    if (n <= 0) return;
-    const uint32_t pl_sa = SharedU32(sw.pl);
-    const uint32_t cp = ncomp > 1 ? uint32_t(8 * mpw * fi.H[1]) : 0u;
-    for (int r = lane >> 2; r < rows; r += 8) {
-        const int y = y0 + r;
-        if (y >= fi.height) break;
-        uint2 yy;
-        asm volatile("ld.shared.v2.u32 {%0, %1}, [%2];" : "=r"(yy.x), "=r"(yy.y) : "r"(pl_sa + uint32_t(r * kWarpW + seg * 8)));
-        Rgb8 o;
-        if (gray) {
-            o.r = o.g = o.b = yy;
-        } else {
-            const uint32_t ca = pl_sa + uint32_t(kWarpLuma) + uint32_t(r >> sy) * cp + uint32_t((seg * 8) >> sx);
-            uint2 uu = make_uint2(0u, 0u), vv = make_uint2(0u, 0u);
-            if (sx == 0) {
-                asm volatile("ld.shared.v2.u32 {%0, %1}, [%2];" : "=r"(uu.x), "=r"(uu.y) : "r"(ca));
-                asm volatile("ld.shared.v2.u32 {%0, %1}, [%2];" : "=r"(vv.x), "=r"(vv.y) : "r"(ca + uint32_t(kWarpChroma)));
-                o = Convert8<0>(yy, uu, vv);
-            } else if (sx == 1) {
-                uu.x = Lds32(ca);
-                vv.x = Lds32(ca + uint32_t(kWarpChroma));
-                o = Convert8<1>(yy, uu, vv);
-            } else {
-                asm volatile("ld.shared.u16 %0, [%1];" : "=r"(uu.x) : "r"(ca));
-                asm volatile("ld.shared.u16 %0, [%1];" : "=r"(vv.x) : "r"(ca + uint32_t(kWarpChroma)));
-                o = Convert8<2>(yy, uu, vv);
-            }
-        }
-        StoreRgb8(fmt, d0, d1, d2, dpitch, y, x, n, o);
-    }
+    int mrow = int(tile >> 16), tx = int(blockIdx.x - fi.tile0) - mrow * int(fi.tiles_x), col = warp;
+    if (a.claim) {
+        uint32_t u = 0;
+        if (lane == 0) u = atomicAdd(a.cursor + (tile & 0xFFFFu), 1u);
+        u = __shfl_sync(0xFFFFFFFFu, u, 0);
+        if (u >= fi.units) return;
+        const uint32_t t = u / kWarpsPerStrip;
+        mrow = int(t / fi.tiles_x);
+        tx = int(t - uint32_t(mrow) * fi.tiles_x);
+        col = int(u % kWarpsPerStrip);
+    }
+    WarpUnit<false>(fi, &s_tab[0][0], s_w[warp], a.entries, a.blk_rec, mrow, tx, col, lane);
 }
 
 }
diff --git a/rocjpeg_b200/csrc/k23_warp.cuh b/rocjpeg_b200/csrc/k23_warp.cuh
--- /dev/null
+++ b/rocjpeg_b200/csrc/k23_warp.cuh
@@ -0,0 +1,187 @@
+#pragma once
+#include <cuda_runtime.h>
+
+#include "idct_core.cuh"
+#include "k3_rows.cuh"
+#include "stages.h"
+
+namespace rjb {
+namespace k23w {
+
+__device__ __forceinline__ uint32_t SharedU32(const void* p) {
+    uint32_t a = uint32_t(__cvta_generic_to_shared(p));
+    asm volatile("mov.u32 %0, %0;" : "+r"(a));
+    return a;
+}
+__device__ __forceinline__ uint32_t Lds32(uint32_t a) {
+    uint32_t v;
+    asm volatile("ld.shared.u32 %0, [%1];" : "=r"(v) : "r"(a));
+    return v;
+}
+__device__ __forceinline__ uint4 Lds128(uint32_t a) {
+    uint4 v;
+    asm volatile("ld.shared.v4.u32 {%0, %1, %2, %3}, [%4];" : "=r"(v.x), "=r"(v.y), "=r"(v.z), "=r"(v.w) : "r"(a));
+    return v;
+}
+__device__ __forceinline__ void Sts32(uint32_t a, uint32_t v) { asm volatile("st.shared.u32 [%0], %1;" ::"r"(a), "r"(v) : "memory"); }
+__device__ __forceinline__ void Sts64(uint32_t a, uint32_t x, uint32_t y) { asm volatile("st.shared.v2.u32 [%0], {%1, %2};" ::"r"(a), "r"(x), "r"(y) : "memory"); }
+__device__ __forceinline__ void Sts128(uint32_t a, uint4 v) {
+    asm volatile("st.shared.v4.u32 [%0], {%1, %2, %3, %4};" ::"r"(a), "r"(v.x), "r"(v.y), "r"(v.z), "r"(v.w) : "memory");
+}
+
+constexpr int kRS = 12, kBS = 104;
+constexpr int kStripW = 256;
+constexpr int kWarpW = 32;
+constexpr int kWarpsPerStrip = kStripW / kWarpW;
+constexpr int kWarpBlocks = 16;
+constexpr int kWarpLuma = kWarpW * 16, kWarpChroma = 256;
+
+struct __align__(16) WarpSmem {
+    int ws[4 * kBS];
+    uint4 meta[kWarpBlocks];
+    uint8_t pl[kWarpLuma + 2 * kWarpChroma];
+};
+
+__device__ __forceinline__ uint32_t TableWord(const uint16_t* qtables, uint32_t qidx, int code) {
+    const int nat = idct::kZigzag[(code + 63) & 63];
+    return uint32_t(code == 1 ? 8 * 4 : ((nat >> 3) * kRS + (nat & 7)) * 4) | (uint32_t(__ldg(qtables + size_t(qidx) * 64 + nat)) << 16);
+}
+
+template <bool kCoherent>
+__device__ __forceinline__ uint32_t LdU32(const uint32_t* p) { return kCoherent ? __ldcg(p) : __ldg(p); }
+template <bool kCoherent>
+__device__ __forceinline__ uint2 LdU64(const uint2* p) { return kCoherent ? __ldcg(p) : __ldg(p); }
+
+template <bool kCoherent>
+__device__ __forceinline__ void WarpUnit(const FusedImage& fi, const uint32_t* tab, WarpSmem& sw, const uint32_t* entries, const BlockRec* blk_rec,
+                                         int mrow, int tx, int col, int lane) {
+    using namespace idct;
+    using namespace k3;
+    const int ncomp = fi.ncomp;
+    const int mpt = fi.mpt, mcus_x = fi.mcus_x;
+    const int mpw = mpt >> 3;
+    const int m0 = tx * mpt + col * mpw, nm = min(mpw, mcus_x - m0);
+    if (nm <= 0) return;
+    int nblocks;
+    {
+        const uint32_t ci0 = fi.comp_info[0], ci1 = ncomp > 1 ? fi.comp_info[1] : 0u, ci2 = ncomp > 2 ? fi.comp_info[2] : 0u;
+        const int nbw0 = nm * int(ci0 & 0xFFu), nbw1 = nm * int(ci1 & 0xFFu), nbw2 = nm * int(ci2 & 0xFFu);
+        const int cnt0 = nbw0 * int((ci0 >> 8) & 0xFFu), cnt1 = nbw1 * int((ci1 >> 8) & 0xFFu), cnt2 = nbw2 * int((ci2 >> 8) & 0xFFu);
+        nblocks = cnt0 + cnt1 + cnt2;
+        if (lane < kWarpBlocks) {
+            uint4 m = make_uint4(0u, 0u, 0u, 0u);
+            if (lane < nblocks) {
+                int g = lane, c = 0, nbw = nbw0;
+                uint32_t ci = ci0;
+                if (g >= cnt0) { g -= cnt0; c = 1; nbw = nbw1; ci = ci1; if (g >= cnt1) { g -= cnt1; c = 2; nbw = nbw2; ci = ci2; } }
+                const int v = g >= nbw ? 1 : 0, bx = g - (v ? nbw : 0);
+                const uint32_t H = ci & 0xFFu;
+                const uint32_t blk = uint32_t(mrow * mcus_x + m0 + (bx >> (ci >> 24))) * uint32_t(fi.bpm) + ((ci >> 16) & 0xFFu) + uint32_t(v) * H + (uint32_t(bx) & (H - 1u));
+                const BlockRec* rp = blk_rec + fi.blk0 + blk;
+                const uint2 r = LdU64<kCoherent>(reinterpret_cast<const uint2*>(rp));
+                uint32_t e0 = blk ? LdU32<kCoherent>(&rp[-1].end) : 0u, e1 = r.x;
+                if (e0 == kNoEntry || e1 == kNoEntry || e1 < e0 || e1 - e0 > 0xFFFFu || e1 > fi.ent_cap) e1 = e0 = 0;
+                const uint32_t pitch = uint32_t(8 * mpw) * H;
+                const uint32_t base = c == 0 ? 0u : uint32_t(kWarpLuma + (c - 1) * kWarpChroma);
+                m.x = e0;
+                m.y = (e1 - e0) | (uint32_t(c) << 16) | (1u << 24);
+                m.z = uint32_t(int(int16_t(r.y & 0xFFFFu)) * int(tab[c * 64 + 1] >> 16));
+                m.w = (base + uint32_t(v * 8) * pitch + uint32_t(bx * 8)) | (pitch << 16);
+            }
+            sw.meta[lane] = m;
+        }
+    }
+    __syncwarp();
+    {
+        const int b = lane >> 3, jj = lane & 7;
+        const uint32_t my_sa = SharedU32(sw.ws) + uint32_t(b * kBS * 4);
+        const uint32_t row_sa = my_sa + uint32_t(jj * kRS * 4), col_sa = my_sa + uint32_t(jj * 4);
+        const uint32_t tab_sa0 = SharedU32(tab), pl_sa = SharedU32(sw.pl);
+        uint32_t meta_sa = SharedU32(sw.meta) + uint32_t(b * 16);
+        const uint32_t* const ent_j = entries + fi.ent0 + jj;
+        const uint32_t meta_end = meta_sa + uint32_t(nblocks * 16);
+#pragma unroll 1
+        for (; meta_sa < meta_end; meta_sa += 4 * 16) {
+            const uint4 m = Lds128(meta_sa);
+            const uint32_t n = m.y & 0xFFFFu;
+            const uint32_t* ep = ent_j + m.x;
+            const uint32_t k = uint32_t(jj);
+            uint32_t e[4];
+#pragma unroll
+            for (int u = 0; u < 4; u++) e[u] = (k + 8u * u < n) ? LdU32<kCoherent>(ep + 8 * u) : 0u;
+            Sts128(row_sa, make_uint4(jj == 0 ? m.z : 0u, 0u, 0u, 0u));
+            Sts128(row_sa + 16, make_uint4(0u, 0u, 0u, 0u));
+            __syncwarp();
+            const uint32_t tab_sa = tab_sa0 + ((m.y >> 8) & 0x300u);
+            auto put = [&](uint32_t en) {
+                const uint32_t tt = Lds32(tab_sa + ((en >> 14) & 0xFCu));
+                Sts32(my_sa + (tt & 0xFFFFu), uint32_t(int(int16_t(en & 0xFFFFu)) * int(tt >> 16)));
+            };
+#pragma unroll
+            for (int u = 0; u < 4; u++)
+                if (k + 8u * u < n) put(e[u]);
+            for (uint32_t kk = k + 32u; kk < n; kk += 8) put(LdU32<kCoherent>(ep + (kk - k)));
+            __syncwarp();
+            int in[8], out[8];
+#pragma unroll
+            for (int r = 0; r < 8; r++) in[r] = int(Lds32(col_sa + uint32_t(r * kRS * 4)));
+            Islow8<11>(in, out, 1 << 10);
+#pragma unroll
+            for (int r = 0; r < 8; r++) Sts32(col_sa + uint32_t(r * kRS * 4), uint32_t(out[r]));
+            __syncwarp();
+            {
+                const uint4 lo = Lds128(row_sa), hi = Lds128(row_sa + 16);
+                in[0] = int(lo.x); in[1] = int(lo.y); in[2] = int(lo.z); in[3] = int(lo.w);
+                in[4] = int(hi.x); in[5] = int(hi.y); in[6] = int(hi.z); in[7] = int(hi.w);
+                Islow8<18>(in, out, (1 << 17) + (128 << 18));
+                if (m.y >> 24) Sts64(pl_sa + (m.w & 0xFFFFu) + uint32_t(jj) * (m.w >> 16), PackSat4(out[0], out[1], out[2], out[3]), PackSat4(out[4], out[5], out[6], out[7]));
+            }
+            __syncwarp();
+        }
+    }
+    const int fmt = fi.fmt;
+    uint8_t* const d0 = fi.dst[0];
+    uint8_t* const d1 = fi.dst[1];
+    uint8_t* const d2 = fi.dst[2];
+    const uint32_t dpitch = fi.dpitch;
+    if (d0 == nullptr || dpitch == 0) return;
+    if (fmt == FMT_RGB_PLANAR && (!d1 || !d2)) return;
+    const bool gray = fi.css == CSS_400;
+    const int sx = fi.sx, sy = fi.sy;
+    const int rows = 8 * fi.vmax, y0 = mrow * rows;
+    const int seg = lane & 3, x = tx * kStripW + col * kWarpW + seg * 8;
+    const int n = fi.width - x;
+    if (n <= 0) return;
+    const uint32_t pl_sa = SharedU32(sw.pl);
+    const uint32_t cp = ncomp > 1 ? uint32_t(8 * mpw * fi.H[1]) : 0u;
+    for (int r = lane >> 2; r < rows; r += 8) {
+        const int y = y0 + r;
+        if (y >= fi.height) break;
+        uint2 yy;
+        asm volatile("ld.shared.v2.u32 {%0, %1}, [%2];" : "=r"(yy.x), "=r"(yy.y) : "r"(pl_sa + uint32_t(r * kWarpW + seg * 8)));
+        Rgb8 o;
+        if (gray) {
+            o.r = o.g = o.b = yy;
+        } else {
+            const uint32_t ca = pl_sa + uint32_t(kWarpLuma) + uint32_t(r >> sy) * cp + uint32_t((seg * 8) >> sx);
+            uint2 uu = make_uint2(0u, 0u), vv = make_uint2(0u, 0u);
+            if (sx == 0) {
+                asm volatile("ld.shared.v2.u32 {%0, %1}, [%2];" : "=r"(uu.x), "=r"(uu.y) : "r"(ca));
+                asm volatile("ld.shared.v2.u32 {%0, %1}, [%2];" : "=r"(vv.x), "=r"(vv.y) : "r"(ca + uint32_t(kWarpChroma)));
+                o = Convert8<0>(yy, uu, vv);
+            } else if (sx == 1) {
+                uu.x = Lds32(ca);
+                vv.x = Lds32(ca + uint32_t(kWarpChroma));
+                o = Convert8<1>(yy, uu, vv);
+            } else {
+                asm volatile("ld.shared.u16 %0, [%1];" : "=r"(uu.x) : "r"(ca));
+                asm volatile("ld.shared.u16 %0, [%1];" : "=r"(vv.x) : "r"(ca + uint32_t(kWarpChroma)));
+                o = Convert8<2>(yy, uu, vv);
+            }
+        }
+        StoreRgb8(fmt, d0, d1, d2, dpitch, y, x, n, o);
+    }
+}
+
+}
+}
diff --git a/rocjpeg_b200/csrc/stages.h b/rocjpeg_b200/csrc/stages.h
--- a/rocjpeg_b200/csrc/stages.h
+++ b/rocjpeg_b200/csrc/stages.h
@@ -107,11 +107,19 @@
     int fusable;
     int dc_image;
     int k1_dc;
+    int early_k23;
+    int early_warps, early_stop;
+    uint32_t* pic_done;
+    uint32_t* ready;
+    uint32_t* cursor;
+    const FusedImage* fused;
+    const uint16_t* qtables;
 };
 
 cudaError_t LaunchK1Sync(const K1Args& a, int round, cudaStream_t stream, int max_iters = 0);
 cudaError_t LaunchK1Write(const K1Args& a, cudaStream_t stream);
 cudaError_t LaunchK1Fused(const K1Args& a, cudaStream_t stream);
+bool EarlyK23Fits(const K1Args& a);
 cudaError_t LaunchK1ClearShort(const K1Args& a, cudaStream_t stream);
 cudaError_t LaunchDcScan(const K1Args& a, cudaStream_t stream);
 
@@ -139,6 +147,9 @@
     const BlockRec* blk_rec;
     int nimages;
     uint32_t total_tiles, total_tiles_w;
+    uint32_t* cursor;
+    int precheck;
+    int claim;
 };
 cudaError_t LaunchK23Fused(const K23Args& a, cudaStream_t stream);
 cudaError_t PreloadK23();
```

Result: slower. 98980, median of 6 (-10.7%).
